# javahedi/SpinDynamics.jl

Hardware: AMD Instinct MI355X
Metric: H|psi> matvecs/s, XXZ L=32 Sz=0 (higher is better)
Workload: dtype c128

## Files before the change

### spindynamics.jl_amd/csrc/kernels_apply.hip

```cpp
#include <hip/hip_runtime.h>

#include <algorithm>
#include <type_traits>

#include "device_common.hpp"


using namespace sd_dev;

namespace {

#ifndef SD_PACK_RING
#define SD_PACK_RING 2
#endif
#ifndef SD_PACK_WGS_PER_CU
#define SD_PACK_WGS_PER_CU 4
#endif
static_assert(SD_PACK_RING >= 2 && SD_PACK_RING <= 4, "ring depth of the packed launch: 2..4 register sets");
static_assert(SD_PACK_WGS_PER_CU >= 2 && SD_PACK_WGS_PER_CU <= 5, "workgroups per CU of the packed launch: 2..5 (95 registers at D = 2)");
template <int NC, int R, int BLOCK, bool FMA, bool PK, bool GEN = false, bool PACK = false>
__global__ __launch_bounds__(BLOCK, (GEN ? 5 : PACK ? SD_PACK_WGS_PER_CU : NC == 2 ? 4 : 5)) void k_apply_tiled(sd_dev_model dm, double *__restrict__ out_,
                                                       const double *__restrict__ psi_, int epi, sd_epi_args ea,
                                                       double *__restrict__ partials, int max_len) {
  using V = typename VT<NC>::type;
  constexpr uint32_t ES = sizeof(V);
  constexpr int WR = R * 64;
  extern __shared__ __attribute__((aligned(16))) unsigned char smem[];
  static_assert(!PACK || (PK && !GEN && R == 4 && BLOCK == 256), "packed launch: four slots of 256 rows, packed tables, chain bonds");
#if SD_PACK_TRACE
  uint64_t trace_t0 = 0;
  if constexpr (PACK) trace_t0 = wall_clock64();
#endif
  constexpr int SLOT_ROWS = WR + 1;
  V *tile = reinterpret_cast<V *>(smem);
  int *lbin = reinterpret_cast<int *>(smem + (size_t)(max_len + 1) * sizeof(V));
  double *red = PACK ? reinterpret_cast<double *>(smem + (size_t)(4 * SLOT_ROWS) * sizeof(V)) : reinterpret_cast<double *>(lbin + 16 * SD_BIN_STRIDE);
  V *tile2 = reinterpret_cast<V *>(red + 32);

  if (ea.batch > 1) {
    const int64_t boff = (int64_t)blockIdx.y * ea.bstride * NC;
    psi_ += boff; out_ += boff;
    if (ea.prev) ea.prev = (const double *)ea.prev + boff;
    if (ea.phi) ea.phi = (const double *)ea.phi + boff;
    if (ea.accv) ea.accv = (double *)ea.accv + boff;
    partials += 2 * (size_t)blockIdx.y * (size_t)dm.n_singles;
    ea.negate = (ea.negate >> blockIdx.y) & 1;
  }
  const V *__restrict__ psi = reinterpret_cast<const V *>(psi_);
  const V *__restrict__ halo = reinterpret_cast<const V *>(ea.halo);
  const int tid = threadIdx.x;
  const int lane = tid & 63;
  int slot_tile = 0, team_wave = 0, team_n = 1, wv = 0;
  bool idle = false;
  if constexpr (PACK) {
    wv = __builtin_amdgcn_readfirstlane(tid >> 6);
    typedef int i4 __attribute__((ext_vector_type(4)));
    const i4 bt = *reinterpret_cast<const i4 *>(dm.blk_tiles + 4 * (size_t)blockIdx.x);
    const int st[4] = {bt.x, bt.y, bt.z, bt.w};
    slot_tile = __builtin_amdgcn_readfirstlane(wv == 0 ? st[0] : wv == 1 ? st[1] : wv == 2 ? st[2] : st[3]);
    team_n = 0;
#pragma unroll
    for (int k = 0; k < 4; ++k) {
      if (st[k] == slot_tile) ++team_n;
      if (st[k] == slot_tile && k < wv) ++team_wave;
    }
    team_wave = __builtin_amdgcn_readfirstlane(team_wave);
    team_n = __builtin_amdgcn_readfirstlane(team_n);
    idle = slot_tile < 0;
    tile += (wv - team_wave) * SLOT_ROWS;
  }
  const int i0 = (PACK ? team_wave : (tid >> 6)) * WR + lane;
  const int tix = PACK ? (idle ? 0 : slot_tile) : blockIdx.x + dm.tile_off;
  const sd_tile_rec rec = dm.single_rec[tix];
  const uint32_t P = rec.prefix;
  const int64_t base = rec.base;
  const int p = dm.p, LS = dm.LS;
  const int len = (PACK && idle) ? 0 : rec.len;
  const int nU = rec.nU;
  const int nn = dm.nn_hops;
  static_assert(!GEN || PK, "general-bond plan: packed tables only");
  const bool need_sig = GEN ? (dm.need_sig_gen != 0) : (!PK || dm.need_sig);

  V own[R];
  uint32_t sig[R];
  typedef unsigned int u4 __attribute__((ext_vector_type(4)));
  u4 pt[PK ? R : 1];
  uint32_t dg[R];
  const uint32_t off0 = (uint32_t)i0 * ES;
  {
    const __amdgpu_buffer_rsrc_t rs = make_rsrc(psi + base, (uint32_t)len * ES);
#pragma unroll
    for (int r = 0; r < R; ++r) buf_load(own[r], rs, off0 + (uint32_t)(r * 64) * ES);
    if (PK && !need_sig && !dm.diag_cache) {
      const __amdgpu_buffer_rsrc_t rg = make_rsrc(dm.suf_dg + rec.suf_off, (uint32_t)len);
#pragma unroll
      for (int r = 0; r < R; ++r) dg[r] = (uint32_t)(unsigned char)__builtin_amdgcn_raw_buffer_load_b8(rg, (uint32_t)i0 + (uint32_t)(r * 64), 0, 0);
    }
    if (need_sig) {
      const __amdgpu_buffer_rsrc_t rsig = make_rsrc(dm.suf_states + rec.suf_off, (uint32_t)len * 2u);
#pragma unroll
      for (int r = 0; r < R; ++r) sig[r] = buf_load_u16(rsig, (uint32_t)i0 * 2u + (uint32_t)(r * 64) * 2u);
    } else {
#pragma unroll
      for (int r = 0; r < R; ++r) sig[r] = 0;
    }
  }

  uint64_t fmask = 0;
  int64_t my_base = -1;
  const uint32_t bitp = p >= 1 ? ((P >> (p - 1)) & 1u) : 0u;
  if (nn > 0 && p >= 1 && !(PACK && idle)) {
    const int b = lane + 1;
    if (b <= p) my_base = dm.far_base[(size_t)tix * (size_t)p + (size_t)lane];
    fmask = __ballot(my_base >= 0);
  }
  const int st_lo = bitp ? nU : 0, st_n = bitp ? len - nU : nU;
  auto get_bond = [&](int ln) {
    FarBond fb;
    fb.base = rl64(my_base, ln); fb.J = dm.hop_J[ln];
    const bool st = ln == p - 1;
    fb.lo = st ? st_lo : 0; fb.n = st ? st_n : len;
    return fb;
  };
  constexpr bool SKIP_DEAD = NC == 1 || BLOCK == 64;
  uint32_t live = 0;
  if (SKIP_DEAD) {
#pragma unroll
    for (int r = 0; r < R; ++r)
      if ((tid & ~63) / 64 * WR + r * 64 < len) live |= 1u << r;
    live = (uint32_t)__builtin_amdgcn_readfirstlane((int)live);
  }
  auto issue = [&](const FarBond &fb, V(&v)[R]) {
    const V *__restrict__ pb = (halo && fb.base >= dm.n_local) ? halo + (fb.base - dm.n_local) : psi + fb.base;
    const __amdgpu_buffer_rsrc_t rs = make_rsrc(pb, (uint32_t)fb.n * ES);
    const uint32_t rel = off0 - (uint32_t)fb.lo * ES;
#pragma unroll
    for (int r = 0; r < R; ++r)
      if (!SKIP_DEAD || ((live >> r) & 1u)) buf_load(v[r], rs, rel + (uint32_t)(r * 64) * ES);
  };

  V va[R], vb[R];
  if (SKIP_DEAD) {
#pragma unroll
    for (int r = 0; r < R; ++r) { va[r] = V{}; vb[r] = V{}; }
  }
  FarBond fa{}, fbb{};
  uint64_t mk = fmask;
  bool have_a = false;
  auto next_lane = [&](uint64_t &m_) { const int ln = __builtin_ctzll(m_); m_ &= m_ - 1; return ln; };
  constexpr int D = PACK ? SD_PACK_RING : 2;
  u4 rq[D][R];
  FarBond fr[D];
  int ring_full = 0, ring_rem = 0;
  auto ring_next = [&]() {
    FarBond fb;
    const bool e = mk == 0;
    const int ln = e ? 0 : __builtin_ctzll(mk);
    mk &= mk - 1;
    fb.base = e ? 0 : rl64(my_base, ln);
    fb.J = 0.0;
    if (!e) fb.J = dm.hop_J[ln];
    const bool st = ln == p - 1;
    fb.lo = st ? st_lo : 0; fb.n = e ? 0 : st ? st_n : len;
    return fb;
  };
  auto ring_issue = [&](const FarBond &fb, u4(&v)[R]) {
    const __amdgpu_buffer_rsrc_t rs = make_rsrc(psi + fb.base, (uint32_t)fb.n * ES);
    const uint32_t rel = off0 - (uint32_t)fb.lo * ES;
#pragma unroll
    for (int r = 0; r < R; ++r) v[r] = __builtin_amdgcn_raw_buffer_load_b128(rs, rel + (uint32_t)(r * 64) * ES, 0, 0);
  };
  auto request_table = [&]() {
    if (PK && (PACK || nn > 0)) {
      const __amdgpu_buffer_rsrc_t rp = make_rsrc(dm.suf_part + 4 * (size_t)rec.suf_off, nn > 0 ? (uint32_t)len * 16u : 0u);
#pragma unroll
      for (int r = 0; r < R; ++r) pt[PK ? r : 0] = __builtin_amdgcn_raw_buffer_load_b128(rp, (uint32_t)i0 * 16u + (uint32_t)(r * 64) * 16u, 0, 0);
    }
  };
  double dd[R];
  auto load_dd = [&]() {
    const __amdgpu_buffer_rsrc_t rd = make_rsrc(dm.diag_cache + base, (uint32_t)len * (uint32_t)sizeof(double));
#pragma unroll
    for (int r = 0; r < R; ++r) buf_load(dd[r], rd, (uint32_t)i0 * (uint32_t)sizeof(double) + (uint32_t)(r * 64) * (uint32_t)sizeof(double));
  };
  if constexpr (PACK) {
    if (dm.diag_cache) load_dd();
    request_table();
    const int nf = __popcll(fmask);
    const int ring_more = nf > D ? nf - D : 0;
    ring_full = ring_more / D;
    ring_rem = ring_more - ring_full * D;
    FarBond fe[D];
#pragma unroll
    for (int j = 0; j < D; ++j) fe[j] = ring_next();
#pragma unroll
    for (int k = 0; k < D; ++k) {
      fr[k] = fe[k];
#pragma unroll
      for (int t = 1; t < D; ++t)
        if (ring_rem == t) fr[k] = fe[(k + t) % D];
      ring_issue(fr[k], rq[k]);
    }
  } else {
    if (mk) { fa = get_bond(next_lane(mk)); issue(fa, va); have_a = true; }
  }

  V acc[R];
  if (dm.diag_cache) {
    if constexpr (!PACK) load_dd();
#pragma unroll
    for (int r = 0; r < R; ++r) acc[r] = vscale(dd[r], own[r]);
  } else if (!need_sig) {
    const int antiP = p >= 2 ? __popc((P ^ (P >> 1)) & ((1u << (p - 1)) - 1u)) : 0;
#pragma unroll
    for (int r = 0; r < R; ++r) {
      int anti = antiP + (int)(dg[r] & 15u) + (p >= 1 ? (int)(bitp ^ (dg[r] >> 4)) : 0);
      if (dm.n_zz_nn == 0) anti = 0;
      acc[r] = vscale(dm.diag_q * (double)(dm.n_zz - 2 * anti), own[r]);
    }
  } else if (dm.diag_mode == 0) {
    const DiagHead dh = diag_head(dm, P, p);
#pragma unroll
    for (int r = 0; r < R; ++r) {
      const uint64_t s = (uint64_t)P | ((uint64_t)sig[r] << p);
      acc[r] = vscale(diag_tail(dm, dh, s, p), own[r]);
    }
  } else {
#pragma unroll
    for (int r = 0; r < R; ++r) {
      const uint64_t s = (uint64_t)P | ((uint64_t)sig[r] << p);
      acc[r] = vscale(diag_of(dm, s), own[r]);
    }
  }
#pragma unroll
  for (int r = 0; r < R; ++r)
    if (i0 + r * 64 < len) tile[1 + i0 + r * 64] = own[r];
  if (PACK ? (lane == 0 && team_wave == 0) : (tid == 0)) tile[0] = V{};
  if (!PK)
    for (int k = tid; k < 16 * SD_BIN_STRIDE; k += BLOCK) {
      int n = k / SD_BIN_STRIDE, kk = k - n * SD_BIN_STRIDE;
      lbin[k] = (int)binom_g(dm, n, kk);
    }

  __syncthreads();
  if constexpr (PACK) {
    auto ring_acc = [&](int k) {
#pragma unroll
      for (int r = 0; r < R; ++r) {
        const u4 q = rq[k][r];
        V v;
        if constexpr (NC == 2) { v.x = __hiloint2double((int)q.y, (int)q.x); v.y = __hiloint2double((int)q.w, (int)q.z); }
        acc[r] = accum<FMA>(acc[r], fr[k].J, v);
      }
    };
    auto ring_step = [&](int k) {
      const FarBond nb = get_bond(next_lane(mk));
      ring_acc(k);
      __builtin_amdgcn_sched_barrier(0);
      fr[k] = nb;
      ring_issue(fr[k], rq[k]);
      __builtin_amdgcn_sched_barrier(0);
    };
#pragma unroll
    for (int k = 1; k < D; ++k)
      if (ring_rem >= D - k) ring_step(k);
#pragma nounroll
    for (int it = 0; it < ring_full; ++it) {
#pragma unroll
      for (int k = 0; k < D; ++k) ring_step(k);
    }
#pragma unroll
    for (int k = 0; k < D; ++k) ring_acc(k);
  } else {
    while (have_a) {
      bool have_b = false;
      if (mk) { fbb = get_bond(next_lane(mk)); issue(fbb, vb); have_b = true; }
#pragma unroll
      for (int r = 0; r < R; ++r) acc[r] = accum<FMA>(acc[r], fa.J, va[r]);
      have_a = false;
      if (!have_b) break;
      if (mk) { fa = get_bond(next_lane(mk)); issue(fa, va); have_a = true; }
#pragma unroll
      for (int r = 0; r < R; ++r) acc[r] = accum<FMA>(acc[r], fbb.J, vb[r]);
    }
  }
  if constexpr (!PACK) request_table();
  const bool wrap = !GEN && !PACK && PK && !(NC == 1 && R == 8) && nn > 0 && dm.wrap_hop == nn;
  bool wrap_on = false;
  if (wrap) {
    const uint32_t Q = P ^ (1u << dm.wrap_pb);
    const int t2q = dm.nup - __popc(Q);
    if (t2q >= 0 && t2q <= LS) {
      wrap_on = true;
      const int64_t qb = dm.addr[Q];
      const int lenq = (int)dm.binom[LS * (SD_MAX_L + 1) + t2q];
      const V *__restrict__ pbq = (halo && qb >= dm.n_local) ? halo + (qb - dm.n_local) : psi + qb;
      const __amdgpu_buffer_rsrc_t rq = make_rsrc(pbq, (uint32_t)lenq * ES);
      for (int c0 = 0; c0 < lenq; c0 += BLOCK * R) {
#pragma unroll
        for (int r = 0; r < R; ++r) buf_load(va[r], rq, off0 + (uint32_t)(c0 + r * 64) * ES);
#pragma unroll
        for (int r = 0; r < R; ++r)
          if (c0 + i0 + r * 64 < lenq) tile2[1 + c0 + i0 + r * 64] = va[r];
      }
      if (tid == 0) tile2[0] = V{};
    }
  }

  struct GBond { int64_t base; uint32_t smask; int pb; int kind; };
  auto gbond = [&](int h) {
    GBond g{0, 0u, 0, -1};
    const int bi = dm.hop_i[h] - 1, bj = dm.hop_j[h] - 1;
    const bool ip = bi < p, jp = bj < p;
    if (ip && jp) {
      if (((P >> bi) ^ (P >> bj)) & 1u) { g.kind = 0; g.base = dm.addr[P ^ (1u << bi) ^ (1u << bj)]; }
    } else if (!ip && !jp) {
      g.kind = 1; g.smask = (1u << (bi - p)) | (1u << (bj - p));
    } else {
      g.pb = ip ? bi : bj;
      g.smask = 1u << ((ip ? bj : bi) - p);
      const uint32_t Q = P ^ (1u << g.pb);
      const int t2q = dm.nup - __popc(Q);
      if (t2q >= 0 && t2q <= LS) { g.kind = 2; g.base = dm.addr[Q]; }
    }
    return g;
  };
  auto gflip = [&](const GBond &g, int r) -> bool {
    if (g.kind == 0) return true;
    if (g.kind == 1) return __popc(sig[r] & g.smask) == 1;
    if (g.kind == 2) return ((P >> g.pb) & 1u) != ((sig[r] & g.smask) ? 1u : 0u);
    return false;
  };
  auto gvalue = [&](const GBond &g, int r) -> V {
    if (g.kind == 1) return tile[1 + dm.suf_rank[sig[r] ^ g.smask]];
    const int64_t idx = g.base + (g.kind == 0 ? (int64_t)(i0 + r * 64) : (int64_t)dm.suf_rank[sig[r] ^ g.smask]);
    return (halo && idx >= dm.n_local) ? halo[idx - dm.n_local] : psi[idx];
  };
  const bool have_g = !GEN && nn < dm.n_hop;
  double gJ = 0.0;
  GBond g0{0, 0u, 0, -1};
  auto request_g0 = [&]() {
    g0 = gbond(nn);
    gJ = dm.hop_J[nn];
#pragma unroll
    for (int r = 0; r < R; ++r) va[r] = (i0 + r * 64 < len && gflip(g0, r)) ? gvalue(g0, r) : V{};
  };
  if (have_g && !PK) request_g0();
  if (nn > 0) {
    if constexpr (PK) {
      const unsigned char *tb = reinterpret_cast<const unsigned char *>(tile);
      constexpr uint32_t SH = NC == 2 ? 4 : 3;
#pragma unroll
      for (int a = 1; a <= 11; ++a) if (a <= LS - 1) {
        const double J = dm.hop_J[p + a - 1];
        const int w = (a - 1) / 3, sh = 10 * ((a - 1) % 3);
        V v[R];
#pragma unroll
        for (int r = 0; r < R; ++r) {
          const u4 q = pt[PK ? r : 0];
          const uint32_t word = w == 0 ? q.x : w == 1 ? q.y : w == 2 ? q.z : q.w;
          const uint32_t ad = ((word >> sh) & 0x3FFu) << SH;
          v[r] = *reinterpret_cast<const V *>(tb + ad);
        }
#pragma unroll
        for (int r = 0; r < R; ++r) acc[r] = accum<FMA>(acc[r], J, v[r]);
      }
    } else {
      uint32_t dw[R];
#pragma unroll
      for (int r = 0; r < R; ++r) dw[r] = sig[r] ^ (sig[r] >> 1);
      for (int a = 1; a <= LS - 1; ++a) {
        const double J = dm.hop_J[p + a - 1];
        const int *brow = lbin + (LS - a - 1) * SD_BIN_STRIDE;
        int d[R];
#pragma unroll
        for (int r = 0; r < R; ++r) d[r] = brow[__popc(sig[r] >> (a + 1))];
        V v[R];
#pragma unroll
        for (int r = 0; r < R; ++r) {
          const bool up = (sig[r] >> (a - 1)) & 1u;
          const bool fl = (dw[r] >> (a - 1)) & 1u;
          const int ip = (i0 + r * 64) + (up ? d[r] : -d[r]);
          v[r] = tile[fl ? ip + 1 : 0];
        }
#pragma unroll
        for (int r = 0; r < R; ++r) acc[r] = accum<FMA>(acc[r], J, v[r]);
      }
    }
  }
  if constexpr (GEN) {
    constexpr uint32_t SH = NC == 2 ? 4 : 3;
    const unsigned char *tb = reinterpret_cast<const unsigned char *>(tile);
    const unsigned char *tb2 = reinterpret_cast<const unsigned char *>(tile2);
    uint32_t ptw[R];
    int cur_word = -1;
    auto gissue = [&](int64_t gbase, V(&v)[R]) {
      const V *__restrict__ pbp = (halo && gbase >= dm.n_local) ? halo + (gbase - dm.n_local) : psi + gbase;
      const __amdgpu_buffer_rsrc_t rs = make_rsrc(pbp, (uint32_t)len * ES);
#pragma unroll
      for (int r = 0; r < R; ++r) buf_load(v[r], rs, off0 + (uint32_t)(r * 64) * ES);
    };
    for (int hb = 0; hb < dm.n_gen; hb += 64) {
      const int nb = dm.n_gen - hb < 64 ? dm.n_gen - hb : 64;
      int64_t base_k = -1;
      sd_gbond gl{-1, 0u, 0, 0, 0.0};
      if (lane < nb) {
        gl = dm.gen[hb + lane];
        if (gl.kind == 0 && __popc(P & gl.pmask) == 1) base_k = dm.addr[P ^ gl.pmask];
      }
      uint64_t todo = __ballot(base_k >= 0);
      int in_a = -1;
      if (todo) { in_a = next_lane(todo); gissue(rl64(base_k, in_a), va); }
#pragma nounroll
      for (int k = 0; k < nb; ++k) {
        sd_gbond gb;
        gb.kind = rl(gl.kind, k); gb.pmask = (uint32_t)rl((int)gl.pmask, k); gb.slot = rl(gl.slot, k); gb.pb = rl(gl.pb, k);
        gb.J = rld(gl.J, k);
        if (gb.kind == 0) {
          if (k == in_a) {
#pragma unroll
            for (int r = 0; r < R; ++r) acc[r] = accum<false>(acc[r], gb.J, va[r]);
            in_a = -1;
            if (todo) { in_a = next_lane(todo); gissue(rl64(base_k, in_a), va); }
          }
        } else if (gb.kind == 1) {
          const int wi = gb.slot / 3, sh = 10 * (gb.slot - 3 * wi);
          if (wi != cur_word) {
            cur_word = wi;
            const int chunk = wi >> 2;
            const __amdgpu_buffer_rsrc_t rp2 = make_rsrc(dm.gen_ss_part + 4 * ((size_t)chunk * (size_t)dm.n_suf_rows + (size_t)rec.suf_off), (uint32_t)len * 16u);
            const uint32_t wo = (uint32_t)(wi & 3) * 4u;
#pragma unroll
            for (int r = 0; r < R; ++r) ptw[r] = (uint32_t)__builtin_amdgcn_raw_buffer_load_b32(rp2, (uint32_t)i0 * 16u + (uint32_t)(r * 64) * 16u + wo, 0, 0);
          }
          V v[R];
#pragma unroll
          for (int r = 0; r < R; ++r) v[r] = *reinterpret_cast<const V *>(tb + ((((ptw[r] >> sh) & 0x3FFu)) << SH));
#pragma unroll
          for (int r = 0; r < R; ++r) acc[r] = accum<false>(acc[r], gb.J, v[r]);
        } else if (gb.kind == 2) {
          const uint32_t Q = P ^ gb.pmask;
          const int t2q = dm.nup - __popc(Q);
          const bool ok = t2q >= 0 && t2q <= LS;
          __syncthreads();
          if (ok) {
            const int64_t qb = dm.addr[Q];
            const int lenq = (int)dm.binom[LS * (SD_MAX_L + 1) + t2q];
            const V *__restrict__ pbq = (halo && qb >= dm.n_local) ? halo + (qb - dm.n_local) : psi + qb;
            const __amdgpu_buffer_rsrc_t rq = make_rsrc(pbq, (uint32_t)lenq * ES);
            for (int c0 = 0; c0 < lenq; c0 += BLOCK * R) {
              V tmp[R];
#pragma unroll
              for (int r = 0; r < R; ++r) buf_load(tmp[r], rq, off0 + (uint32_t)(c0 + r * 64) * ES);
#pragma unroll
              for (int r = 0; r < R; ++r)
                if (c0 + i0 + r * 64 < lenq) tile2[1 + c0 + i0 + r * 64] = tmp[r];
            }
            if (tid == 0) tile2[0] = V{};
          }
          __syncthreads();
          if (ok) {
            const __amdgpu_buffer_rsrc_t rm = make_rsrc(dm.mix_part + ((size_t)gb.slot * (size_t)dm.n_suf_rows + (size_t)rec.suf_off), (uint32_t)len * 2u);
            const uint32_t bpb = (P >> gb.pb) & 1u;
            uint32_t w16[R];
#pragma unroll
            for (int r = 0; r < R; ++r) w16[r] = buf_load_u16(rm, (uint32_t)i0 * 2u + (uint32_t)(r * 64) * 2u);
#pragma unroll
            for (int r = 0; r < R; ++r) {
              const bool has = (w16[r] >> 15) != bpb;
              const uint32_t ad = has ? ((w16[r] & 0x3FFu) << SH) : 0u;
              acc[r] = accum<false>(acc[r], gb.J, *reinterpret_cast<const V *>(tb2 + ad));
            }
          }
        }
      }
    }
  }
  if (wrap) {
    __syncthreads();
    if (wrap_on) {
      const double Jw = dm.hop_J[nn];
      const uint32_t bpb = (P >> dm.wrap_pb) & 1u;
      const unsigned char *tb2 = reinterpret_cast<const unsigned char *>(tile2);
      constexpr uint32_t SH = NC == 2 ? 4 : 3;
#pragma unroll
      for (int r = 0; r < R; ++r) {
        const uint32_t w3 = pt[PK ? r : 0].w;
        const bool has = ((w3 >> 30) & 1u) != bpb;
        const uint32_t ad = has ? (((w3 >> 20) & 0x3FFu) << SH) : 0u;
        acc[r] = accum<false>(acc[r], Jw, *reinterpret_cast<const V *>(tb2 + ad));
      }
    }
  }
  if (have_g) {
    if (!wrap) {
      if (PK) request_g0();
#pragma unroll
      for (int r = 0; r < R; ++r)
        if (gflip(g0, r)) acc[r] = accum<false>(acc[r], gJ, va[r]);
    }
    for (int h = nn + 1; h < dm.n_hop; ++h) {
      const GBond g = gbond(h);
      if (g.kind < 0) continue;
      const double J = dm.hop_J[h];
#pragma unroll
      for (int r = 0; r < R; ++r)
        if (i0 + r * 64 < len && gflip(g, r)) acc[r] = accum<false>(acc[r], J, gvalue(g, r));
    }
  }

  EpiSums sums{0.0, 0.0};
#pragma unroll
  for (int r = 0; r < R; ++r) {
    const int i = i0 + r * 64;
    if (i < len) epilogue<NC>(epi, ea, base + i, acc[r], tile[1 + i], out_, sums);
  }
  if (epi_has_sums(epi)) {
    double a = sums.s0, b = sums.s1;
    if constexpr (PACK) {
      for (int off = 32; off > 0; off >>= 1) {
        a += __shfl_down(a, off, 64);
        b += __shfl_down(b, off, 64);
      }
      if (lane == 0) { red[2 * wv] = a; red[2 * wv + 1] = b; }
      __syncthreads();
      if (lane == 0 && team_wave == 0 && !idle) {
        double x = 0.0, y = 0.0;
        for (int w = 0; w < team_n; ++w) { x += red[2 * (wv + w)]; y += red[2 * (wv + w) + 1]; }
        partials[2 * (size_t)tix] = x; partials[2 * (size_t)tix + 1] = y;
      }
    } else {
      block_reduce2(a, b, red);
      if (tid == 0) { partials[2 * (size_t)tix] = a; partials[2 * (size_t)tix + 1] = b; }
    }
  }
#if SD_PACK_TRACE
  if constexpr (PACK) {
    if (dm.pack_trace && tid == 0 && blockIdx.y == 0) {
      __builtin_amdgcn_s_waitcnt(0);
      uint64_t *rec_t = dm.pack_trace + 3 * (size_t)blockIdx.x;
      rec_t[0] = trace_t0;
      rec_t[1] = wall_clock64();
      rec_t[2] = (uint64_t)(__builtin_amdgcn_s_getreg((3 << 11) | 20) & 15u);
    }
  }
#endif
}

template <int NC, bool FMA>
__global__ __launch_bounds__(256, 4) void k_apply_fulltile(sd_dev_model dm, double *__restrict__ out_,
                                                        const double *__restrict__ psi_, int epi, sd_epi_args ea,
                                                        double *__restrict__ partials) {
  using V = typename VT<NC>::type;
  constexpr uint32_t ES = sizeof(V);
  constexpr int R = 4, BLOCK = 256;
  extern __shared__ __attribute__((aligned(16))) unsigned char smem[];
  const int LF = dm.full_ls, TL = 1 << LF;
  V *tile = reinterpret_cast<V *>(smem);
  double *red = reinterpret_cast<double *>(smem + (size_t)(TL + 1) * sizeof(V));
  const V *__restrict__ psi = reinterpret_cast<const V *>(psi_);
  const V *__restrict__ halo = reinterpret_cast<const V *>(ea.halo);
  const int tid = threadIdx.x, lane = tid & 63;
  uint32_t T = blockIdx.x;
  if (gridDim.x >= 512 && (gridDim.x & 255u) == 0) {
    const uint32_t x = T & 7u, j = T >> 3, g = j >> 5, i = j & 31u;
    T = (g << 8) + (x << 5) + i;
  }
  const int64_t base = (int64_t)T << LF;
  const uint32_t Tg = T + (uint32_t)(dm.row_lo >> LF);
  const int64_t gbase = (int64_t)Tg << LF;
  const int nn = dm.nn_hops;

  V own[R];
  uint32_t ioff[R];
  {
    const __amdgpu_buffer_rsrc_t rs = make_rsrc(psi + base, (uint32_t)TL * ES);
#pragma unroll
    for (int r = 0; r < R; ++r) { ioff[r] = (uint32_t)(tid + r * BLOCK) * ES; buf_load(own[r], rs, ioff[r]); }
  }
  uint64_t fmask = 0;
  int64_t my_base = 0;
  double my_J = 0.0;
  int my_lo = 0, my_n = TL;
  if (nn > 0) {
    const int a = LF + lane;
    bool fl = false;
    if (a <= dm.L - 1) {
      if (lane == 0) {
        const int t = (int)(T & 1u);
        my_lo = (1 - t) * (TL / 2); my_n = TL / 2;
        my_base = ((int64_t)(T ^ 1u) << LF) + (TL / 2 - my_lo);
        fl = true;
      } else {
        const int b = a - LF - 1;
        fl = ((Tg >> b) ^ (Tg >> (b + 1))) & 1u;
        const uint32_t Tp = Tg ^ (3u << b);
        const int tb = dm.L - LF - dm.fs_dbits;
        const uint32_t q = Tp >> tb;
        const int64_t at_peer = (int64_t)(Tp & ((1u << tb) - 1u)) << LF;
        my_base = at_peer;
        if (q != (Tg >> tb)) {
          int64_t ho = 0, plo = 0;
#pragma unroll
          for (int q2 = 0; q2 < SD_FS_MAX_RANKS; ++q2)
            if ((uint32_t)q2 == q) { ho = dm.fs_halo_off[q2]; plo = dm.fs_peer_lo[q2]; }
          my_base = dm.n_local + ho + at_peer - plo;
        }
      }
      my_J = dm.hop_J[a - 1];
    }
    fmask = __ballot(fl);
  }
  auto get_bond = [&](int ln) {
    FarBond fb;
    fb.base = rl64(my_base, ln); fb.J = rld(my_J, ln);
    fb.lo = rl(my_lo, ln); fb.n = rl(my_n, ln);
    return fb;
  };
  auto issue = [&](const FarBond &fb, V(&v)[R]) {
    const V *__restrict__ pb = (halo && fb.base >= dm.n_local) ? halo + (fb.base - dm.n_local) : psi + fb.base;
    const __amdgpu_buffer_rsrc_t rs = make_rsrc(pb, (uint32_t)fb.n * ES);
    const uint32_t lo_b = (uint32_t)fb.lo * ES;
#pragma unroll
    for (int r = 0; r < R; ++r) buf_load(v[r], rs, ioff[r] - lo_b);
  };
  V va[R], vb[R];
  FarBond fa{}, fbb{};
  uint64_t mk = fmask;
  bool have_a = false;
  auto next_lane = [&](uint64_t &m_) { const int ln = __builtin_ctzll(m_); m_ &= m_ - 1; return ln; };
  if (mk) { fa = get_bond(next_lane(mk)); issue(fa, va); have_a = true; }

  V acc[R];
#pragma unroll
  for (int r = 0; r < R; ++r) {
    acc[r] = vscale(diag_of(dm, (uint64_t)gbase + (uint64_t)(tid + r * BLOCK)), own[r]);
    tile[tid + r * BLOCK] = own[r];
  }
  if (tid == 0) tile[TL] = V{};
  __syncthreads();

  const int n_in = nn > 0 ? LF - 1 : 0;
  for (int a = 1; a <= n_in; ++a) {
    const double J = dm.hop_J[a - 1];
    V v[R];
#pragma unroll
    for (int r = 0; r < R; ++r) {
      const int i = tid + r * BLOCK;
      const bool fl = ((i >> (a - 1)) ^ (i >> a)) & 1;
      v[r] = tile[fl ? (i ^ (3 << (a - 1))) : TL];
    }
#pragma unroll
    for (int r = 0; r < R; ++r) acc[r] = accum<FMA>(acc[r], J, v[r]);
  }
  while (have_a) {
    bool have_b = false;
    if (mk) { fbb = get_bond(next_lane(mk)); issue(fbb, vb); have_b = true; }
#pragma unroll
    for (int r = 0; r < R; ++r) acc[r] = accum<FMA>(acc[r], fa.J, va[r]);
    have_a = false;
    if (!have_b) break;
    if (mk) { fa = get_bond(next_lane(mk)); issue(fa, va); have_a = true; }
#pragma unroll
    for (int r = 0; r < R; ++r) acc[r] = accum<FMA>(acc[r], fbb.J, vb[r]);
  }
  for (int h = nn; h < dm.n_hop; ++h) {
    const int bi = dm.hop_i[h] - 1, bj = dm.hop_j[h] - 1;
    const double J = dm.hop_J[h];
#pragma unroll
    for (int r = 0; r < R; ++r) {
      const uint64_t s = (uint64_t)gbase + (uint64_t)(tid + r * BLOCK);
      if (((s >> bi) ^ (s >> bj)) & 1) acc[r] = accum<false>(acc[r], J, psi[s ^ ((uint64_t)1 << bi) ^ ((uint64_t)1 << bj)]);
    }
  }
  EpiSums sums{0.0, 0.0};
#pragma unroll
  for (int r = 0; r < R; ++r) {
    const int i = tid + r * BLOCK;
    epilogue<NC>(epi, ea, base + i, acc[r], tile[i], out_, sums);
  }
  if (epi_has_sums(epi)) {
    double a = sums.s0, b = sums.s1;
    block_reduce2(a, b, red);
    if (tid == 0) { partials[2 * (size_t)blockIdx.x] = a; partials[2 * (size_t)blockIdx.x + 1] = b; }
  }
}

template <int NC>
__global__ __launch_bounds__(256) void k_apply_generic(sd_dev_model dm, double *__restrict__ out_,
                                                       const double *__restrict__ psi_, int epi, sd_epi_args ea,
                                                       double *__restrict__ partials) {
  using V = typename VT<NC>::type;
  __shared__ double red[32];
  __shared__ int64_t lb[64 * 64];
  const V *__restrict__ psi = reinterpret_cast<const V *>(psi_);
  const bool full = dm.nup < 0;
  const int L = dm.L;
  if (!full) {
    for (int i = threadIdx.x; i < 64 * 64; i += blockDim.x) {
      const int n = i >> 6, k = i & 63;
      lb[i] = (n <= L && k <= n) ? dm.binom[n * (SD_MAX_L + 1) + k] : 0;
    }
    __syncthreads();
  }
  auto bl = [&](int n, int k) -> int64_t { return (k < 0 || k > n) ? 0 : lb[(n << 6) + k]; };
  auto unrank_l = [&](int64_t idx) {
    uint64_t s = 0;
    int r = dm.nup;
    for (int k = 1; k <= L && r > 0; ++k) {
      const int64_t c = bl(L - k, r - 1);
      if (idx < c) { s |= (uint64_t)1 << (k - 1); --r; }
      else idx -= c;
    }
    return s;
  };
  auto rank_l = [&](uint64_t s) {
    int64_t idx = 0;
    int r = dm.nup;
    for (int k = 1; k <= L && r > 0; ++k) {
      if ((s >> (k - 1)) & 1) --r;
      else idx += bl(L - k, r - 1);
    }
    return idx;
  };
  const int nn = full ? 0 : dm.nn_hops;
  EpiSums sums{0.0, 0.0};
  const int64_t stride = (int64_t)gridDim.x * blockDim.x;
  for (int64_t idx = (int64_t)blockIdx.x * blockDim.x + threadIdx.x; idx < dm.N; idx += stride) {
    const uint64_t s = full ? (uint64_t)idx : unrank_l(idx);
    const V own = psi[idx];
    V acc = vscale(diag_of(dm, s), own);
    for (int b = 1; b <= nn; ++b)
      if (((s >> (b - 1)) ^ (s >> b)) & 1) {
        const int64_t d = lb[((L - b - 1) << 6) + __popcll(s >> (b + 1))];
        const int64_t nidx = ((s >> (b - 1)) & 1) ? idx + d : idx - d;
        acc = vadd_mul(acc, dm.hop_J[b - 1], psi[nidx]);
      }
    for (int h = nn; h < dm.n_hop; ++h) {
      const int bi = dm.hop_i[h] - 1, bj = dm.hop_j[h] - 1;
      if (((s >> bi) ^ (s >> bj)) & 1) {
        const uint64_t s2 = s ^ ((uint64_t)1 << bi) ^ ((uint64_t)1 << bj);
        const int64_t nidx = full ? (int64_t)s2 : rank_l(s2);
        acc = vadd_mul(acc, dm.hop_J[h], psi[nidx]);
      }
    }
    epilogue<NC>(epi, ea, idx, acc, own, out_, sums);
  }
  if (epi_has_sums(epi)) {
    double a = sums.s0, b = sums.s1;
    block_reduce2(a, b, red);
    if (threadIdx.x == 0) { partials[2 * (size_t)blockIdx.x] = a; partials[2 * (size_t)blockIdx.x + 1] = b; }
  }
}

template <int NC, int LPT>
__global__ __launch_bounds__(256) void k_apply_short(sd_dev_model dm, double *__restrict__ out_, const double *__restrict__ psi_, int epi,
                                                     sd_epi_args ea, double *__restrict__ partials, int first, int count) {
  using V = typename VT<NC>::type;
  __shared__ int64_t lb[64 * 64];
  if (ea.batch > 1) {
    const int64_t boff = (int64_t)blockIdx.y * ea.bstride * NC;
    psi_ += boff; out_ += boff;
    if (ea.prev) ea.prev = (const double *)ea.prev + boff;
    if (ea.phi) ea.phi = (const double *)ea.phi + boff;
    if (ea.accv) ea.accv = (double *)ea.accv + boff;
    partials += 2 * (size_t)blockIdx.y * (size_t)dm.n_singles;
    ea.negate = (ea.negate >> blockIdx.y) & 1;
  }
  const V *__restrict__ psi = reinterpret_cast<const V *>(psi_);
  const int L = dm.L, p = dm.p;
  for (int i = threadIdx.x; i < 64 * 64; i += blockDim.x) {
    const int n = i >> 6, k = i & 63;
    lb[i] = (n <= L && k <= n) ? dm.binom[n * (SD_MAX_L + 1) + k] : 0;
  }
  __syncthreads();
  auto bl = [&](int n, int k) -> int64_t { return (k < 0 || k > n) ? 0 : lb[(n << 6) + k]; };
  auto rank_l = [&](uint64_t s) {
    int64_t idx = 0;
    int r = dm.nup;
    for (int k = 1; k <= L && r > 0; ++k) {
      if ((s >> (k - 1)) & 1) --r;
      else idx += bl(L - k, r - 1);
    }
    return idx;
  };
  constexpr int TPB = 256 / LPT;
  const int i = threadIdx.x % LPT;
  const int nn = dm.nn_hops;
  const int sweeps = (count + (int)gridDim.x * TPB - 1) / ((int)gridDim.x * TPB);
  for (int sw = 0; sw < sweeps; ++sw) {
    const int g = (sw * (int)gridDim.x + (int)blockIdx.x) * TPB + (int)threadIdx.x / LPT;
    const bool have_tile = g < count;
    const int tix = first + (have_tile ? g : 0);
    const sd_tile_rec rec = dm.single_rec[tix];
    EpiSums sums{0.0, 0.0};
    if (have_tile && i < rec.len) {
      const int64_t idx = rec.base + i;
      const uint64_t s = (uint64_t)rec.prefix | ((uint64_t)dm.suf_states[rec.suf_off + i] << p);
      const V own = psi[idx];
      V acc = vscale(dm.diag_cache ? dm.diag_cache[idx] : diag_of(dm, s), own);
      for (int b = 1; b <= nn; ++b)
        if (((s >> (b - 1)) ^ (s >> b)) & 1) {
          const int64_t d = lb[((L - b - 1) << 6) + __popcll(s >> (b + 1))];
          const int64_t nidx = ((s >> (b - 1)) & 1) ? idx + d : idx - d;
          acc = vadd_mul(acc, dm.hop_J[b - 1], psi[nidx]);
        }
      for (int h = nn; h < dm.n_hop; ++h) {
        const int bi = dm.hop_i[h] - 1, bj = dm.hop_j[h] - 1;
        if (((s >> bi) ^ (s >> bj)) & 1) {
          const uint64_t s2 = s ^ ((uint64_t)1 << bi) ^ ((uint64_t)1 << bj);
          acc = vadd_mul(acc, dm.hop_J[h], psi[rank_l(s2)]);
        }
      }
      epilogue<NC>(epi, ea, idx, acc, own, out_, sums);
    }
    if (epi_has_sums(epi)) {
      double a = sums.s0, b = sums.s1;
      if (LPT > 1)
        for (int off = LPT / 2; off > 0; off >>= 1) {
          a += __shfl_down(a, off, LPT);
          b += __shfl_down(b, off, LPT);
        }
      if (have_tile && i == 0) { partials[2 * (size_t)tix] = a; partials[2 * (size_t)tix + 1] = b; }
    }
  }
}

template <int NC>
__global__ __launch_bounds__(256) void k_epilogue_only(int epi, sd_epi_args ea, int64_t n, double *out_,
                                                       const double *hpsi_, const double *__restrict__ psi_,
                                                       double *__restrict__ partials) {
  using V = typename VT<NC>::type;
  __shared__ double red[32];
  const V *hpsi = reinterpret_cast<const V *>(hpsi_);
  const V *__restrict__ psi = reinterpret_cast<const V *>(psi_);
  EpiSums sums{0.0, 0.0};
  const int64_t stride = (int64_t)gridDim.x * blockDim.x;
  for (int64_t i = (int64_t)blockIdx.x * blockDim.x + threadIdx.x; i < n; i += stride) {
    const V acc = hpsi[i], own = psi[i];
    epilogue<NC>(epi, ea, i, acc, own, out_, sums);
  }
  if (epi_has_sums(epi)) {
    double a = sums.s0, b = sums.s1;
    block_reduce2(a, b, red);
    if (threadIdx.x == 0) { partials[2 * (size_t)blockIdx.x] = a; partials[2 * (size_t)blockIdx.x + 1] = b; }
  }
}

__global__ __launch_bounds__(1024) void k_reduce_pairs(const double *__restrict__ partials, int64_t n,
                                                       double *__restrict__ scalars, int64_t dstride) {
  __shared__ double red[32];
  partials += 2 * (size_t)blockIdx.x * (size_t)n;
  scalars += (size_t)blockIdx.x * (size_t)dstride;
  double a = 0.0, b = 0.0;
  for (int64_t i = threadIdx.x; i < n; i += blockDim.x) { a += partials[2 * i]; b += partials[2 * i + 1]; }
  block_reduce2(a, b, red);
  if (threadIdx.x == 0) { scalars[0] = a; scalars[1] = b; }
}

__global__ __launch_bounds__(256) void k_reduce_pairs_stage(const double *__restrict__ partials, int64_t n, int64_t chunk,
                                                            double *__restrict__ stage) {
  __shared__ double red[32];
  const int64_t lo = (int64_t)blockIdx.x * chunk, hi = lo + chunk < n ? lo + chunk : n;
  const double2 *__restrict__ p2 = reinterpret_cast<const double2 *>(partials);
  double a = 0.0, b = 0.0;
  for (int64_t i = lo + threadIdx.x; i < hi; i += blockDim.x) { const double2 v = p2[i]; a += v.x; b += v.y; }
  block_reduce2(a, b, red);
  if (threadIdx.x == 0) { stage[2 * blockIdx.x] = a; stage[2 * blockIdx.x + 1] = b; }
}

}
int sd_reduce_pairs(sd_ctx *ctx, int64_t n, double *dst) {
  if (!dst) dst = ctx->d_scalars;
  const double *src = ctx->d_partials;
  if (n > 16384) {
    double *stage = ctx->d_partials + 2 * n;
    const int64_t chunk = (n + SD_RED_STAGE_BLOCKS - 1) / SD_RED_STAGE_BLOCKS;
    hipLaunchKernelGGL(k_reduce_pairs_stage, dim3(SD_RED_STAGE_BLOCKS), dim3(256), 0, ctx->stream, src, n, chunk, stage);
    SD_HIP(ctx, hipGetLastError());
    src = stage; n = SD_RED_STAGE_BLOCKS;
  }
  hipLaunchKernelGGL(k_reduce_pairs, dim3(1), dim3(1024), 0, ctx->stream, src, n, dst, (int64_t)0);
  SD_HIP(ctx, hipGetLastError());
  return SD_OK;
}
int sd_reduce_pairs_batched(sd_ctx *ctx, int64_t n, int batch, double *dst, int64_t dstride) {
  if (!dst || n > 16384 || batch < 1) return sd_set_err(ctx, SD_EINTERNAL, "bad batched reduction");
  hipLaunchKernelGGL(k_reduce_pairs, dim3((unsigned)batch), dim3(1024), 0, ctx->stream, ctx->d_partials, n, dst, dstride);
  SD_HIP(ctx, hipGetLastError());
  return SD_OK;
}
int sd_launch_epilogue_only(sd_ctx *ctx, int dtype, int64_t n, void *out, const void *hpsi, const void *psi, int epi,
                            const sd_epi_args &ea_in) {
  const bool sums = (epi == SD_EPI_DOT || epi == SD_EPI_KPM || epi == SD_EPI_RESCALE_DOT);
  sd_epi_args ea = ea_in;
  ea.stream_hint = 0;
  if (n <= 0) {
    if (sums) SD_HIP(ctx, hipMemsetAsync(ea.sums_dst ? ea.sums_dst : ctx->d_scalars, 0, 2 * sizeof(double), ctx->stream));
    return SD_OK;
  }
  const int64_t nb = std::min<int64_t>((n + 255) / 256, 4096);
  if (sums) { int rc = sd_ensure_partials(ctx, 2 * (size_t)nb + 2 * SD_RED_STAGE_BLOCKS); if (rc) return rc; }
  if (dtype == SD_C128)
    hipLaunchKernelGGL(k_epilogue_only<2>, dim3((unsigned)nb), dim3(256), 0, ctx->stream, epi, ea, n, (double *)out,
                       (const double *)hpsi, (const double *)psi, ctx->d_partials);
  else
    hipLaunchKernelGGL(k_epilogue_only<1>, dim3((unsigned)nb), dim3(256), 0, ctx->stream, epi, ea, n, (double *)out,
                       (const double *)hpsi, (const double *)psi, ctx->d_partials);
  SD_HIP(ctx, hipGetLastError());
  if (sums) return sd_reduce_pairs(ctx, nb, ea.sums_dst);
  return SD_OK;
}
namespace {

template <int NC, int R, int BLOCK, bool FMA, bool PK, bool GEN = false, bool PACK = false>
int launch_tiled_cfg(sd_ctx *ctx, const sd_dev_model &dm, int nt, size_t shmem, double *out, const double *psi, int epi,
                     const sd_epi_args &ea, int max_len) {
  void (*kern)(sd_dev_model, double *, const double *, int, sd_epi_args, double *, int) = k_apply_tiled<NC, R, BLOCK, FMA, PK, GEN, PACK>;
  if (shmem > 48 * 1024)
    SD_HIP(ctx, hipFuncSetAttribute((const void *)kern, hipFuncAttributeMaxDynamicSharedMemorySize, (int)shmem));
  hipLaunchKernelGGL(kern, dim3(nt, ea.batch > 1 ? ea.batch : 1), dim3(BLOCK), shmem, ctx->stream, dm, out, psi, epi, ea, ctx->d_partials, max_len);
  SD_HIP(ctx, hipGetLastError());
  return SD_OK;
}

template <int NC, bool FMA>
int launch_tiled(sd_ctx *ctx, const sd_dev_model &dm, int nt, int cls, size_t shmem, double *out, const double *psi, int epi,
                 const sd_epi_args &ea, int max_len) {
  constexpr int R = 4;
  if ((64 << cls) * R < max_len) return sd_set_err(ctx, SD_EINTERNAL, "tile longer than its workgroup can hold");
  if (!dm.suf_part) {
    switch (cls) {
      case 3: return launch_tiled_cfg<NC, R, 512, FMA, false>(ctx, dm, nt, shmem, out, psi, epi, ea, max_len);
      case 4: return launch_tiled_cfg<NC, R, 1024, FMA, false>(ctx, dm, nt, shmem, out, psi, epi, ea, max_len);
    }
    return sd_set_err(ctx, SD_EINTERNAL, "bad tile length class for a plan without the packed partner table");
  }
  if (dm.n_gen > 0)
    switch (cls) {
      case 0: return launch_tiled_cfg<NC, R, 64, FMA, true, true>(ctx, dm, nt, shmem, out, psi, epi, ea, max_len);
      case 1: return launch_tiled_cfg<NC, R, 128, FMA, true, true>(ctx, dm, nt, shmem, out, psi, epi, ea, max_len);
      case 2: return launch_tiled_cfg<NC, R, 256, FMA, true, true>(ctx, dm, nt, shmem, out, psi, epi, ea, max_len);
      default: return sd_set_err(ctx, SD_EINTERNAL, "bad tile length class");
    }
  constexpr bool F8 = NC == 1;
  switch (cls) {
    case 0: return launch_tiled_cfg<NC, R, 64, FMA, true>(ctx, dm, nt, shmem, out, psi, epi, ea, max_len);
    case 1: return launch_tiled_cfg<NC, F8 ? 8 : R, F8 ? 64 : 128, FMA, true>(ctx, dm, nt, shmem, out, psi, epi, ea, max_len);
    case 2: return launch_tiled_cfg<NC, F8 ? 8 : R, F8 ? 128 : 256, FMA, true>(ctx, dm, nt, shmem, out, psi, epi, ea, max_len);
  }
  return sd_set_err(ctx, SD_EINTERNAL, "bad tile length class");
}

}

int sd_launch_apply(sd_ctx *ctx, const sd_model *m, int dtype, void *out, const void *psi, int epi,
                    const sd_epi_args &ea_in, int part) {
  if (!m->dev_ready) return sd_set_err(ctx, SD_EARG, "model has no device tables (created without a context)");
  if (dtype != SD_F64 && dtype != SD_C128) return sd_set_err(ctx, SD_EARG, "dtype must be SD_F64 or SD_C128");
  const bool sums = (epi == SD_EPI_DOT || epi == SD_EPI_KPM || epi == SD_EPI_RESCALE_DOT);
  sd_dev_model dm = m->dm;
  sd_epi_args ea = ea_in;
  ea.stream_hint = 3;
  if (dm.n_local == 0) {
    if (sums) SD_HIP(ctx, hipMemsetAsync(ea.sums_dst ? ea.sums_dst : ctx->d_scalars, 0, 2 * sizeof(double), ctx->stream));
    return SD_OK;
  }
  if (ea.no_reduce && (m->p < 0 || part != 0)) return sd_set_err(ctx, SD_EINTERNAL, "unreduced sums: whole tiled plans only");
  if (ea.batch > 1 && (m->p < 0 || m->nranks != 1 || part != 0 || dm.n_singles > 16384 || (sums && !ea.sums_dst && !ea.no_reduce)))
    return sd_set_err(ctx, SD_EINTERNAL, "batched apply: unsharded tiled plans with at most 16384 tiles only");
  if (m->p >= 0) {
    int nt = dm.n_singles;
    if (part == 1) nt = dm.n_interior;
    else if (part == 2) nt = dm.n_singles - dm.n_interior;
    if (sums) { int rc = sd_ensure_partials(ctx, 2 * (size_t)dm.n_singles * (size_t)std::max(ea.batch, 1) + 2 * SD_RED_STAGE_BLOCKS); if (rc) return rc; }
    const int max_len = m->max_tile_len;
    const size_t esz = dtype == SD_C128 ? 16 : 8;
    int rc = SD_OK;
    if (nt > 0) {
      const bool packed = part == 0 && dtype == SD_C128 && dm.n_blk > 0;
      if (packed) {
        constexpr size_t LDS_CU = 160 * 1024, WGS = SD_PACK_WGS_PER_CU;
        const size_t need = (size_t)4 * 257 * esz + 32 * sizeof(double) + 16;
        const size_t shmem = WGS >= 6 ? need : std::max(need, ((LDS_CU / WGS + LDS_CU / (WGS + 1)) / 2) & ~(size_t)255);
        rc = m->hop_pow2 ? launch_tiled_cfg<2, 4, 256, true, true, false, true>(ctx, dm, dm.n_blk, shmem, (double *)out, (const double *)psi, epi, ea, 1024)
                         : launch_tiled_cfg<2, 4, 256, false, true, false, true>(ctx, dm, dm.n_blk, shmem, (double *)out, (const double *)psi, epi, ea, 1024);
      }
      const int s0 = part == 2 ? SD_N_LEN_CLASS : 0, s1 = packed ? s0 : part == 1 ? SD_N_LEN_CLASS : 2 * SD_N_LEN_CLASS;
      for (int sg = s0; sg < s1 && rc == SD_OK; ++sg) {
        const int cnt = m->seg_off[sg + 1] - m->seg_off[sg];
        if (cnt <= 0) continue;
        const int cls = m->seg_cls[sg];
        const int seg_max = std::min(max_len, (64 << cls) * 4);
        size_t shmem = (size_t)(seg_max + 1) * esz + 16 * SD_BIN_STRIDE * sizeof(int) + 32 * sizeof(double) + 16;
        if ((dm.wrap_hop >= 0 && dm.wrap_hop == dm.nn_hops) || dm.n_gen_mixed > 0) shmem += (size_t)(m->max_tile_len_all + 1) * esz;
        dm.tile_off = m->seg_off[sg];
        if (dtype == SD_C128)
          rc = m->hop_pow2 ? launch_tiled<2, true>(ctx, dm, cnt, cls, shmem, (double *)out, (const double *)psi, epi, ea, seg_max)
                           : launch_tiled<2, false>(ctx, dm, cnt, cls, shmem, (double *)out, (const double *)psi, epi, ea, seg_max);
        else
          rc = m->hop_pow2 ? launch_tiled<1, true>(ctx, dm, cnt, cls, shmem, (double *)out, (const double *)psi, epi, ea, seg_max)
                           : launch_tiled<1, false>(ctx, dm, cnt, cls, shmem, (double *)out, (const double *)psi, epi, ea, seg_max);
      }
      if (rc) return rc;
      if (dm.n_short > 0 && part == 0) {
        const unsigned by = ea.batch > 1 ? (unsigned)ea.batch : 1u;
        auto blocks = [](int tiles, int per_block) { return (unsigned)std::min(4096, std::max(1, (tiles + per_block - 1) / per_block)); };
        const int n16 = dm.n_short_multi, n1 = dm.n_short - dm.n_short_multi;
        if (n16 > 0) {
          if (dtype == SD_C128) hipLaunchKernelGGL((k_apply_short<2, 16>), dim3(blocks(n16, 16), by), dim3(256), 0, ctx->stream, dm, (double *)out, (const double *)psi, epi, ea, ctx->d_partials, dm.short_off, n16);
          else hipLaunchKernelGGL((k_apply_short<1, 16>), dim3(blocks(n16, 16), by), dim3(256), 0, ctx->stream, dm, (double *)out, (const double *)psi, epi, ea, ctx->d_partials, dm.short_off, n16);
        }
        if (n1 > 0) {
          if (dtype == SD_C128) hipLaunchKernelGGL((k_apply_short<2, 1>), dim3(blocks(n1, 256), by), dim3(256), 0, ctx->stream, dm, (double *)out, (const double *)psi, epi, ea, ctx->d_partials, dm.short_off + n16, n1);
          else hipLaunchKernelGGL((k_apply_short<1, 1>), dim3(blocks(n1, 256), by), dim3(256), 0, ctx->stream, dm, (double *)out, (const double *)psi, epi, ea, ctx->d_partials, dm.short_off + n16, n1);
        }
        SD_HIP(ctx, hipGetLastError());
      }
    }
    if (sums && part != 1 && !ea.no_reduce) {
      int rc2 = ea.batch > 1 ? sd_reduce_pairs_batched(ctx, (int64_t)dm.n_singles, ea.batch, ea.sums_dst, ea.sums_bstride)
                             : sd_reduce_pairs(ctx, (int64_t)dm.n_singles, ea.sums_dst);
      if (rc2) return rc2;
    }
  } else if (m->full_ls > 0) {
    if (part == 1) return SD_OK;
    const int64_t nb = dm.n_local >> m->full_ls;
    if (sums) { int rc = sd_ensure_partials(ctx, 2 * (size_t)nb + 2 * SD_RED_STAGE_BLOCKS); if (rc) return rc; }
    const size_t esz = dtype == SD_C128 ? 16 : 8;
    const size_t shmem = (((size_t)1 << m->full_ls) + 1) * esz + 32 * sizeof(double) + 16;
    void (*kf)(sd_dev_model, double *, const double *, int, sd_epi_args, double *) =
        dtype == SD_C128 ? (m->hop_pow2 ? k_apply_fulltile<2, true> : k_apply_fulltile<2, false>)
                         : (m->hop_pow2 ? k_apply_fulltile<1, true> : k_apply_fulltile<1, false>);
    hipLaunchKernelGGL(kf, dim3((unsigned)nb), dim3(256), shmem, ctx->stream, dm, (double *)out, (const double *)psi, epi, ea,
                       ctx->d_partials);
    SD_HIP(ctx, hipGetLastError());
    if (sums) {
      int rc2 = sd_reduce_pairs(ctx, (int64_t)nb, ea.sums_dst);
      if (rc2) return rc2;
    }
  } else {
    int64_t nb = (dm.N + 255) / 256;
    if (nb > 8192) nb = 8192;
    if (sums) { int rc = sd_ensure_partials(ctx, 2 * (size_t)nb + 2 * SD_RED_STAGE_BLOCKS); if (rc) return rc; }
    if (dtype == SD_C128)
      hipLaunchKernelGGL(k_apply_generic<2>, dim3((unsigned)nb), dim3(256), 0, ctx->stream, dm, (double *)out,
                         (const double *)psi, epi, ea, ctx->d_partials);
    else
      hipLaunchKernelGGL(k_apply_generic<1>, dim3((unsigned)nb), dim3(256), 0, ctx->stream, dm, (double *)out,
                         (const double *)psi, epi, ea, ctx->d_partials);
    SD_HIP(ctx, hipGetLastError());
    if (sums) {
      int rc2 = sd_reduce_pairs(ctx, (int64_t)nb, ea.sums_dst);
      if (rc2) return rc2;
    }
  }
  return SD_OK;
}
```

Before: 105.6.

## Specialize packed tiled kernel body by live row-group count per wave

The tiled kernel body now lives in a self-included section, so it can be instantiated several times with a compile-time row count R. In the packed launch, each wave computes how many 64-row groups of its slot are live and dispatches to a body with R=4 or R=2 (or R=3, depending on SD_PACK_BODIES). This avoids issuing loads and accumulations for dead row groups. Hop amplitudes in the packed path are also read through the constant address space. The cost is larger code and possible divergence in register allocation between bodies, plus some added compile complexity.

```diff
diff --git a/profiles/live_groups.py b/profiles/live_groups.py
--- /dev/null
+++ b/profiles/live_groups.py
@@ -0,0 +1,141 @@
+#!/usr/bin/env python3
+import os
+import sys
+from collections import Counter
+from math import comb
+
+sys.path.insert(0, os.path.dirname(os.path.abspath(__file__)))
+from orbit_key import deal, orbit_key, tile_costs
+
+QUAD_BLOCKS, CAP_TENTHS, DEAL_COST, RUN = 2, 78, "slots", 3
+RING = 2
+SLOT_GROUPS, GROUP_ROWS = 4, 64
+
+
+def tile_len(P, nup, LS):
+    t = nup - bin(P).count("1")
+    return comb(LS, t) if 0 <= t <= LS else 0
+
+
+def tile_base(P, L, p, nup):
+    idx, r = 0, nup
+    for k in range(1, p + 1):
+        if r <= 0:
+            break
+        if (P >> (k - 1)) & 1:
+            r -= 1
+        else:
+            idx += comb(L - k, r - 1)
+    return idx
+
+
+def list_length(P, p, nup, LS):
+    n = bin((P ^ (P >> 1)) & ((1 << (p - 1)) - 1)).count("1") if p >= 2 else 0
+    t = nup - bin(P).count("1")
+    bitp = (P >> (p - 1)) & 1
+    tq = t + 1 if bitp else t - 1
+    nU = comb(LS - 1, t - 1) if t >= 1 else 0
+    mine = comb(LS, t) - nU if bitp else nU
+    return n + (1 if 0 <= tq <= LS and mine > 0 else 0)
+
+
+def queues(L, nup, LS=12):
+    p = L - LS
+    tiles = sorted((P for P in range(1 << p) if tile_len(P, nup, LS) > 0), key=lambda P: tile_base(P, L, p, nup))
+    first, keys = {}, []
+    for P in tiles:
+        rep, mem, _ = orbit_key(P, p, QUAD_BLOCKS, CAP_TENTHS)
+        keys.append((first.setdefault(rep, len(first)), mem))
+    idx = sorted(range(len(tiles)), key=lambda k: keys[k])
+    orbits, members = [], []
+    for k in idx:
+        if not members or keys[k][0] != keys[members[-1][0]][0]:
+            members.append([])
+            orbits.append([0, 0, 0, 0, 0])
+        members[-1].append(k)
+        orbits[-1][0] += 1
+        for n, c in enumerate(tile_costs(tiles[k], p, LS, nup, QUAD_BLOCKS, CAP_TENTHS)):
+            orbits[-1][1 + n] += c
+    q = [[] for _ in range(8)]
+    for mem, x in zip(members, deal([tuple(o) for o in orbits], DEAL_COST, RUN)):
+        q[x].extend(tiles[k] for k in mem)
+    return q
+
+
+def blocks(L, nup, LS=12):
+    out = []
+    for queue in queues(L, nup, LS):
+        cur = []
+        for P in queue:
+            s = (tile_len(P, nup, LS) + 255) // 256
+            if len(cur) + s > 4:
+                out.append(tuple(cur + [-1] * (4 - len(cur))))
+                cur = []
+            cur += [P] * s
+        if cur:
+            out.append(tuple(cur + [-1] * (4 - len(cur))))
+    return out
+
+
+def waves(L, nup, LS=12):
+    p = L - LS
+    out = []
+    for blk in blocks(L, nup, LS):
+        for w, P in enumerate(blk):
+            if P < 0:
+                out.append((0, 0, 0))
+                continue
+            team_wave = w - blk.index(P)
+            ln = tile_len(P, nup, LS)
+            live = min(SLOT_GROUPS, max(0, -(-(ln - team_wave * SLOT_GROUPS * GROUP_ROWS) // GROUP_ROWS)))
+            out.append((ln, live, list_length(P, p, nup, LS)))
+    return out
+
+
+def groups_run(live, bodies):
+    live = max(live, 1)
+    return SLOT_GROUPS if bodies == 1 else live if bodies == 4 else (2 if live <= 2 else 4)
+
+
+def vmem_reads(ln, live, nf, bodies):
+    g = groups_run(live, bodies)
+    return (3 + max(nf, RING)) * g + (1 if ln > 0 else 0)
+
+
+def count(L, nup, LS=12):
+    ws = waves(L, nup, LS)
+    by_len = {}
+    for ln, live, _ in ws:
+        if ln == 0:
+            continue
+        t = by_len.setdefault(ln, [0, 0, 0])
+        t[1] += SLOT_GROUPS
+        t[2] += live
+    for ln, t in by_len.items():
+        t[0] = t[1] // (SLOT_GROUPS * ((ln + 255) // 256))
+    return {"by_len": {ln: tuple(t) for ln, t in by_len.items()},
+            "idle": sum(1 for w in ws if w[0] == 0),
+            "body": Counter(max(w[1], 1) for w in ws),
+            "groups": {b: sum(groups_run(w[1], b) for w in ws) for b in (1, 2, 4)},
+            "vmem": {b: sum(vmem_reads(*w, b) for w in ws) for b in (1, 2, 4)}}
+
+
+if __name__ == "__main__":
+    L = int(sys.argv[1]) if len(sys.argv) > 1 else 32
+    nup = int(sys.argv[2]) if len(sys.argv) > 2 else L // 2
+    LS = int(sys.argv[3]) if len(sys.argv) > 3 else 12
+    c = count(L, nup, LS)
+    print(f"L={L} nup={nup} LS={LS}: packed launch, {sum(c['body'].values())} wave slots, {c['idle']} idle")
+    print("| tile rows | slots | groups issued / live per tile | tiles | dead groups |")
+    print("|---:|---:|---:|---:|---:|")
+    for ln in sorted(c["by_len"], reverse=True):
+        tiles, issued, live = c["by_len"][ln]
+        print(f"| {ln} | {(ln + 255) // 256} | {issued // tiles} / {live // tiles} | {tiles} | {issued - live} |")
+    issued = sum(t[1] for t in c["by_len"].values())
+    live = sum(t[2] for t in c["by_len"].values())
+    print(f"row groups of tiles: {issued} issued, {live} live, {issued - live} dead ({100.0 * (issued - live) / issued:.2f} %);"
+          f" idle slots add {SLOT_GROUPS * c['idle']} issued groups before, {c['idle']} now")
+    print("waves by live groups (idle slots under 1):", dict(sorted(c["body"].items())))
+    for b, name in ((1, "before (every wave four groups)"), (4, "four bodies"), (2, "two bodies (<= 2, 4)")):
+        print(f"{name:34s}: {c['groups'][b]:>10d} groups run, {c['vmem'][b]:>11d} vector-memory read wave-instructions"
+              f" ({100.0 * (c['vmem'][b] - c['vmem'][1]) / c['vmem'][1]:+.2f} %)")
diff --git a/spindynamics.jl_amd/csrc/kernels_apply.hip b/spindynamics.jl_amd/csrc/kernels_apply.hip
--- a/spindynamics.jl_amd/csrc/kernels_apply.hip
+++ b/spindynamics.jl_amd/csrc/kernels_apply.hip
@@ -1,3 +1,4 @@
+#ifndef SD_TILED_BODY_PASS
 #include <hip/hip_runtime.h>
 
 #include <algorithm>
@@ -16,17 +17,26 @@
 #ifndef SD_PACK_WGS_PER_CU
 #define SD_PACK_WGS_PER_CU 4
 #endif
+template <bool CONST_AS>
+__device__ __forceinline__ double hop_amp(const double *__restrict__ J, int h) {
+  if constexpr (CONST_AS) return ((const __attribute__((address_space(4))) double *)J)[h];
+  else return J[h];
+}
+#ifndef SD_PACK_BODIES
+#define SD_PACK_BODIES 2
+#endif
+static_assert(SD_PACK_BODIES == 1 || SD_PACK_BODIES == 2 || SD_PACK_BODIES == 4, "bodies of the packed launch: 1, 2 or 4");
 static_assert(SD_PACK_RING >= 2 && SD_PACK_RING <= 4, "ring depth of the packed launch: 2..4 register sets");
 static_assert(SD_PACK_WGS_PER_CU >= 2 && SD_PACK_WGS_PER_CU <= 5, "workgroups per CU of the packed launch: 2..5 (95 registers at D = 2)");
-template <int NC, int R, int BLOCK, bool FMA, bool PK, bool GEN = false, bool PACK = false>
+template <int NC, int RW, int BLOCK, bool FMA, bool PK, bool GEN = false, bool PACK = false>
 __global__ __launch_bounds__(BLOCK, (GEN ? 5 : PACK ? SD_PACK_WGS_PER_CU : NC == 2 ? 4 : 5)) void k_apply_tiled(sd_dev_model dm, double *__restrict__ out_,
                                                        const double *__restrict__ psi_, int epi, sd_epi_args ea,
                                                        double *__restrict__ partials, int max_len) {
   using V = typename VT<NC>::type;
   constexpr uint32_t ES = sizeof(V);
-  constexpr int WR = R * 64;
+  constexpr int WR = RW * 64;
   extern __shared__ __attribute__((aligned(16))) unsigned char smem[];
-  static_assert(!PACK || (PK && !GEN && R == 4 && BLOCK == 256), "packed launch: four slots of 256 rows, packed tables, chain bonds");
+  static_assert(!PACK || (PK && !GEN && RW == 4 && BLOCK == 256), "packed launch: four slots of 256 rows, packed tables, chain bonds");
 #if SD_PACK_TRACE
   uint64_t trace_t0 = 0;
   if constexpr (PACK) trace_t0 = wall_clock64();
@@ -81,459 +91,28 @@
   static_assert(!GEN || PK, "general-bond plan: packed tables only");
   const bool need_sig = GEN ? (dm.need_sig_gen != 0) : (!PK || dm.need_sig);
 
-  V own[R];
-  uint32_t sig[R];
-  typedef unsigned int u4 __attribute__((ext_vector_type(4)));
-  u4 pt[PK ? R : 1];
-  uint32_t dg[R];
-  const uint32_t off0 = (uint32_t)i0 * ES;
-  {
-    const __amdgpu_buffer_rsrc_t rs = make_rsrc(psi + base, (uint32_t)len * ES);
-#pragma unroll
-    for (int r = 0; r < R; ++r) buf_load(own[r], rs, off0 + (uint32_t)(r * 64) * ES);
-    if (PK && !need_sig && !dm.diag_cache) {
-      const __amdgpu_buffer_rsrc_t rg = make_rsrc(dm.suf_dg + rec.suf_off, (uint32_t)len);
-#pragma unroll
-      for (int r = 0; r < R; ++r) dg[r] = (uint32_t)(unsigned char)__builtin_amdgcn_raw_buffer_load_b8(rg, (uint32_t)i0 + (uint32_t)(r * 64), 0, 0);
-    }
-    if (need_sig) {
-      const __amdgpu_buffer_rsrc_t rsig = make_rsrc(dm.suf_states + rec.suf_off, (uint32_t)len * 2u);
-#pragma unroll
-      for (int r = 0; r < R; ++r) sig[r] = buf_load_u16(rsig, (uint32_t)i0 * 2u + (uint32_t)(r * 64) * 2u);
+#define SD_TILED_BODY_PASS 1
+  if constexpr (!PACK) {
+    constexpr int R = RW;
+#include "kernels_apply.hip"
+  } else {
+    int n_live = (len - team_wave * WR + 63) >> 6;
+    n_live = __builtin_amdgcn_readfirstlane(n_live < 1 ? 1 : n_live > RW ? RW : n_live);
+    if (SD_PACK_BODIES == 1 || n_live == 4 || (SD_PACK_BODIES == 2 && n_live == 3)) {
+      constexpr int R = 4;
+#include "kernels_apply.hip"
+    } else if (SD_PACK_BODIES == 4 && n_live == 3) {
+      constexpr int R = 3;
+#include "kernels_apply.hip"
+    } else if (SD_PACK_BODIES == 2 || n_live == 2) {
+      constexpr int R = 2;
+#include "kernels_apply.hip"
     } else {
-#pragma unroll
-      for (int r = 0; r < R; ++r) sig[r] = 0;
-    }
-  }
-
-  uint64_t fmask = 0;
-  int64_t my_base = -1;
-  const uint32_t bitp = p >= 1 ? ((P >> (p - 1)) & 1u) : 0u;
-  if (nn > 0 && p >= 1 && !(PACK && idle)) {
-    const int b = lane + 1;
-    if (b <= p) my_base = dm.far_base[(size_t)tix * (size_t)p + (size_t)lane];
-    fmask = __ballot(my_base >= 0);
-  }
-  const int st_lo = bitp ? nU : 0, st_n = bitp ? len - nU : nU;
-  auto get_bond = [&](int ln) {
-    FarBond fb;
-    fb.base = rl64(my_base, ln); fb.J = dm.hop_J[ln];
-    const bool st = ln == p - 1;
-    fb.lo = st ? st_lo : 0; fb.n = st ? st_n : len;
-    return fb;
-  };
-  constexpr bool SKIP_DEAD = NC == 1 || BLOCK == 64;
-  uint32_t live = 0;
-  if (SKIP_DEAD) {
-#pragma unroll
-    for (int r = 0; r < R; ++r)
-      if ((tid & ~63) / 64 * WR + r * 64 < len) live |= 1u << r;
-    live = (uint32_t)__builtin_amdgcn_readfirstlane((int)live);
-  }
-  auto issue = [&](const FarBond &fb, V(&v)[R]) {
-    const V *__restrict__ pb = (halo && fb.base >= dm.n_local) ? halo + (fb.base - dm.n_local) : psi + fb.base;
-    const __amdgpu_buffer_rsrc_t rs = make_rsrc(pb, (uint32_t)fb.n * ES);
-    const uint32_t rel = off0 - (uint32_t)fb.lo * ES;
-#pragma unroll
-    for (int r = 0; r < R; ++r)
-      if (!SKIP_DEAD || ((live >> r) & 1u)) buf_load(v[r], rs, rel + (uint32_t)(r * 64) * ES);
-  };
-
-  V va[R], vb[R];
-  if (SKIP_DEAD) {
-#pragma unroll
-    for (int r = 0; r < R; ++r) { va[r] = V{}; vb[r] = V{}; }
-  }
-  FarBond fa{}, fbb{};
-  uint64_t mk = fmask;
-  bool have_a = false;
-  auto next_lane = [&](uint64_t &m_) { const int ln = __builtin_ctzll(m_); m_ &= m_ - 1; return ln; };
-  constexpr int D = PACK ? SD_PACK_RING : 2;
-  u4 rq[D][R];
-  FarBond fr[D];
-  int ring_full = 0, ring_rem = 0;
-  auto ring_next = [&]() {
-    FarBond fb;
-    const bool e = mk == 0;
-    const int ln = e ? 0 : __builtin_ctzll(mk);
-    mk &= mk - 1;
-    fb.base = e ? 0 : rl64(my_base, ln);
-    fb.J = 0.0;
-    if (!e) fb.J = dm.hop_J[ln];
-    const bool st = ln == p - 1;
-    fb.lo = st ? st_lo : 0; fb.n = e ? 0 : st ? st_n : len;
-    return fb;
-  };
-  auto ring_issue = [&](const FarBond &fb, u4(&v)[R]) {
-    const __amdgpu_buffer_rsrc_t rs = make_rsrc(psi + fb.base, (uint32_t)fb.n * ES);
-    const uint32_t rel = off0 - (uint32_t)fb.lo * ES;
-#pragma unroll
-    for (int r = 0; r < R; ++r) v[r] = __builtin_amdgcn_raw_buffer_load_b128(rs, rel + (uint32_t)(r * 64) * ES, 0, 0);
-  };
-  auto request_table = [&]() {
-    if (PK && (PACK || nn > 0)) {
-      const __amdgpu_buffer_rsrc_t rp = make_rsrc(dm.suf_part + 4 * (size_t)rec.suf_off, nn > 0 ? (uint32_t)len * 16u : 0u);
-#pragma unroll
-      for (int r = 0; r < R; ++r) pt[PK ? r : 0] = __builtin_amdgcn_raw_buffer_load_b128(rp, (uint32_t)i0 * 16u + (uint32_t)(r * 64) * 16u, 0, 0);
-    }
-  };
-  double dd[R];
-  auto load_dd = [&]() {
-    const __amdgpu_buffer_rsrc_t rd = make_rsrc(dm.diag_cache + base, (uint32_t)len * (uint32_t)sizeof(double));
-#pragma unroll
-    for (int r = 0; r < R; ++r) buf_load(dd[r], rd, (uint32_t)i0 * (uint32_t)sizeof(double) + (uint32_t)(r * 64) * (uint32_t)sizeof(double));
-  };
-  if constexpr (PACK) {
-    if (dm.diag_cache) load_dd();
-    request_table();
-    const int nf = __popcll(fmask);
-    const int ring_more = nf > D ? nf - D : 0;
-    ring_full = ring_more / D;
-    ring_rem = ring_more - ring_full * D;
-    FarBond fe[D];
-#pragma unroll
-    for (int j = 0; j < D; ++j) fe[j] = ring_next();
-#pragma unroll
-    for (int k = 0; k < D; ++k) {
-      fr[k] = fe[k];
-#pragma unroll
-      for (int t = 1; t < D; ++t)
-        if (ring_rem == t) fr[k] = fe[(k + t) % D];
-      ring_issue(fr[k], rq[k]);
-    }
-  } else {
-    if (mk) { fa = get_bond(next_lane(mk)); issue(fa, va); have_a = true; }
-  }
-
-  V acc[R];
-  if (dm.diag_cache) {
-    if constexpr (!PACK) load_dd();
-#pragma unroll
-    for (int r = 0; r < R; ++r) acc[r] = vscale(dd[r], own[r]);
-  } else if (!need_sig) {
-    const int antiP = p >= 2 ? __popc((P ^ (P >> 1)) & ((1u << (p - 1)) - 1u)) : 0;
-#pragma unroll
-    for (int r = 0; r < R; ++r) {
-      int anti = antiP + (int)(dg[r] & 15u) + (p >= 1 ? (int)(bitp ^ (dg[r] >> 4)) : 0);
-      if (dm.n_zz_nn == 0) anti = 0;
-      acc[r] = vscale(dm.diag_q * (double)(dm.n_zz - 2 * anti), own[r]);
-    }
-  } else if (dm.diag_mode == 0) {
-    const DiagHead dh = diag_head(dm, P, p);
-#pragma unroll
-    for (int r = 0; r < R; ++r) {
-      const uint64_t s = (uint64_t)P | ((uint64_t)sig[r] << p);
-      acc[r] = vscale(diag_tail(dm, dh, s, p), own[r]);
-    }
-  } else {
-#pragma unroll
-    for (int r = 0; r < R; ++r) {
-      const uint64_t s = (uint64_t)P | ((uint64_t)sig[r] << p);
-      acc[r] = vscale(diag_of(dm, s), own[r]);
-    }
-  }
-#pragma unroll
-  for (int r = 0; r < R; ++r)
-    if (i0 + r * 64 < len) tile[1 + i0 + r * 64] = own[r];
-  if (PACK ? (lane == 0 && team_wave == 0) : (tid == 0)) tile[0] = V{};
-  if (!PK)
-    for (int k = tid; k < 16 * SD_BIN_STRIDE; k += BLOCK) {
-      int n = k / SD_BIN_STRIDE, kk = k - n * SD_BIN_STRIDE;
-      lbin[k] = (int)binom_g(dm, n, kk);
-    }
-
-  __syncthreads();
-  if constexpr (PACK) {
-    auto ring_acc = [&](int k) {
-#pragma unroll
-      for (int r = 0; r < R; ++r) {
-        const u4 q = rq[k][r];
-        V v;
-        if constexpr (NC == 2) { v.x = __hiloint2double((int)q.y, (int)q.x); v.y = __hiloint2double((int)q.w, (int)q.z); }
-        acc[r] = accum<FMA>(acc[r], fr[k].J, v);
-      }
-    };
-    auto ring_step = [&](int k) {
-      const FarBond nb = get_bond(next_lane(mk));
-      ring_acc(k);
-      __builtin_amdgcn_sched_barrier(0);
-      fr[k] = nb;
-      ring_issue(fr[k], rq[k]);
-      __builtin_amdgcn_sched_barrier(0);
-    };
-#pragma unroll
-    for (int k = 1; k < D; ++k)
-      if (ring_rem >= D - k) ring_step(k);
-#pragma nounroll
-    for (int it = 0; it < ring_full; ++it) {
-#pragma unroll
-      for (int k = 0; k < D; ++k) ring_step(k);
-    }
-#pragma unroll
-    for (int k = 0; k < D; ++k) ring_acc(k);
-  } else {
-    while (have_a) {
-      bool have_b = false;
-      if (mk) { fbb = get_bond(next_lane(mk)); issue(fbb, vb); have_b = true; }
-#pragma unroll
-      for (int r = 0; r < R; ++r) acc[r] = accum<FMA>(acc[r], fa.J, va[r]);
-      have_a = false;
-      if (!have_b) break;
-      if (mk) { fa = get_bond(next_lane(mk)); issue(fa, va); have_a = true; }
-#pragma unroll
-      for (int r = 0; r < R; ++r) acc[r] = accum<FMA>(acc[r], fbb.J, vb[r]);
-    }
-  }
-  if constexpr (!PACK) request_table();
-  const bool wrap = !GEN && !PACK && PK && !(NC == 1 && R == 8) && nn > 0 && dm.wrap_hop == nn;
-  bool wrap_on = false;
-  if (wrap) {
-    const uint32_t Q = P ^ (1u << dm.wrap_pb);
-    const int t2q = dm.nup - __popc(Q);
-    if (t2q >= 0 && t2q <= LS) {
-      wrap_on = true;
-      const int64_t qb = dm.addr[Q];
-      const int lenq = (int)dm.binom[LS * (SD_MAX_L + 1) + t2q];
-      const V *__restrict__ pbq = (halo && qb >= dm.n_local) ? halo + (qb - dm.n_local) : psi + qb;
-      const __amdgpu_buffer_rsrc_t rq = make_rsrc(pbq, (uint32_t)lenq * ES);
-      for (int c0 = 0; c0 < lenq; c0 += BLOCK * R) {
-#pragma unroll
-        for (int r = 0; r < R; ++r) buf_load(va[r], rq, off0 + (uint32_t)(c0 + r * 64) * ES);
-#pragma unroll
-        for (int r = 0; r < R; ++r)
-          if (c0 + i0 + r * 64 < lenq) tile2[1 + c0 + i0 + r * 64] = va[r];
-      }
-      if (tid == 0) tile2[0] = V{};
-    }
-  }
-
-  struct GBond { int64_t base; uint32_t smask; int pb; int kind; };
-  auto gbond = [&](int h) {
-    GBond g{0, 0u, 0, -1};
-    const int bi = dm.hop_i[h] - 1, bj = dm.hop_j[h] - 1;
-    const bool ip = bi < p, jp = bj < p;
-    if (ip && jp) {
-      if (((P >> bi) ^ (P >> bj)) & 1u) { g.kind = 0; g.base = dm.addr[P ^ (1u << bi) ^ (1u << bj)]; }
-    } else if (!ip && !jp) {
-      g.kind = 1; g.smask = (1u << (bi - p)) | (1u << (bj - p));
-    } else {
-      g.pb = ip ? bi : bj;
-      g.smask = 1u << ((ip ? bj : bi) - p);
-      const uint32_t Q = P ^ (1u << g.pb);
-      const int t2q = dm.nup - __popc(Q);
-      if (t2q >= 0 && t2q <= LS) { g.kind = 2; g.base = dm.addr[Q]; }
-    }
-    return g;
-  };
-  auto gflip = [&](const GBond &g, int r) -> bool {
-    if (g.kind == 0) return true;
-    if (g.kind == 1) return __popc(sig[r] & g.smask) == 1;
-    if (g.kind == 2) return ((P >> g.pb) & 1u) != ((sig[r] & g.smask) ? 1u : 0u);
-    return false;
-  };
-  auto gvalue = [&](const GBond &g, int r) -> V {
-    if (g.kind == 1) return tile[1 + dm.suf_rank[sig[r] ^ g.smask]];
-    const int64_t idx = g.base + (g.kind == 0 ? (int64_t)(i0 + r * 64) : (int64_t)dm.suf_rank[sig[r] ^ g.smask]);
-    return (halo && idx >= dm.n_local) ? halo[idx - dm.n_local] : psi[idx];
-  };
-  const bool have_g = !GEN && nn < dm.n_hop;
-  double gJ = 0.0;
-  GBond g0{0, 0u, 0, -1};
-  auto request_g0 = [&]() {
-    g0 = gbond(nn);
-    gJ = dm.hop_J[nn];
-#pragma unroll
-    for (int r = 0; r < R; ++r) va[r] = (i0 + r * 64 < len && gflip(g0, r)) ? gvalue(g0, r) : V{};
-  };
-  if (have_g && !PK) request_g0();
-  if (nn > 0) {
-    if constexpr (PK) {
-      const unsigned char *tb = reinterpret_cast<const unsigned char *>(tile);
-      constexpr uint32_t SH = NC == 2 ? 4 : 3;
-#pragma unroll
-      for (int a = 1; a <= 11; ++a) if (a <= LS - 1) {
-        const double J = dm.hop_J[p + a - 1];
-        const int w = (a - 1) / 3, sh = 10 * ((a - 1) % 3);
-        V v[R];
-#pragma unroll
-        for (int r = 0; r < R; ++r) {
-          const u4 q = pt[PK ? r : 0];
-          const uint32_t word = w == 0 ? q.x : w == 1 ? q.y : w == 2 ? q.z : q.w;
-          const uint32_t ad = ((word >> sh) & 0x3FFu) << SH;
-          v[r] = *reinterpret_cast<const V *>(tb + ad);
-        }
-#pragma unroll
-        for (int r = 0; r < R; ++r) acc[r] = accum<FMA>(acc[r], J, v[r]);
-      }
-    } else {
-      uint32_t dw[R];
-#pragma unroll
-      for (int r = 0; r < R; ++r) dw[r] = sig[r] ^ (sig[r] >> 1);
-      for (int a = 1; a <= LS - 1; ++a) {
-        const double J = dm.hop_J[p + a - 1];
-        const int *brow = lbin + (LS - a - 1) * SD_BIN_STRIDE;
-        int d[R];
-#pragma unroll
-        for (int r = 0; r < R; ++r) d[r] = brow[__popc(sig[r] >> (a + 1))];
-        V v[R];
-#pragma unroll
-        for (int r = 0; r < R; ++r) {
-          const bool up = (sig[r] >> (a - 1)) & 1u;
-          const bool fl = (dw[r] >> (a - 1)) & 1u;
-          const int ip = (i0 + r * 64) + (up ? d[r] : -d[r]);
-          v[r] = tile[fl ? ip + 1 : 0];
-        }
-#pragma unroll
-        for (int r = 0; r < R; ++r) acc[r] = accum<FMA>(acc[r], J, v[r]);
-      }
-    }
-  }
-  if constexpr (GEN) {
-    constexpr uint32_t SH = NC == 2 ? 4 : 3;
-    const unsigned char *tb = reinterpret_cast<const unsigned char *>(tile);
-    const unsigned char *tb2 = reinterpret_cast<const unsigned char *>(tile2);
-    uint32_t ptw[R];
-    int cur_word = -1;
-    auto gissue = [&](int64_t gbase, V(&v)[R]) {
-      const V *__restrict__ pbp = (halo && gbase >= dm.n_local) ? halo + (gbase - dm.n_local) : psi + gbase;
-      const __amdgpu_buffer_rsrc_t rs = make_rsrc(pbp, (uint32_t)len * ES);
-#pragma unroll
-      for (int r = 0; r < R; ++r) buf_load(v[r], rs, off0 + (uint32_t)(r * 64) * ES);
-    };
-    for (int hb = 0; hb < dm.n_gen; hb += 64) {
-      const int nb = dm.n_gen - hb < 64 ? dm.n_gen - hb : 64;
-      int64_t base_k = -1;
-      sd_gbond gl{-1, 0u, 0, 0, 0.0};
-      if (lane < nb) {
-        gl = dm.gen[hb + lane];
-        if (gl.kind == 0 && __popc(P & gl.pmask) == 1) base_k = dm.addr[P ^ gl.pmask];
-      }
-      uint64_t todo = __ballot(base_k >= 0);
-      int in_a = -1;
-      if (todo) { in_a = next_lane(todo); gissue(rl64(base_k, in_a), va); }
-#pragma nounroll
-      for (int k = 0; k < nb; ++k) {
-        sd_gbond gb;
-        gb.kind = rl(gl.kind, k); gb.pmask = (uint32_t)rl((int)gl.pmask, k); gb.slot = rl(gl.slot, k); gb.pb = rl(gl.pb, k);
-        gb.J = rld(gl.J, k);
-        if (gb.kind == 0) {
-          if (k == in_a) {
-#pragma unroll
-            for (int r = 0; r < R; ++r) acc[r] = accum<false>(acc[r], gb.J, va[r]);
-            in_a = -1;
-            if (todo) { in_a = next_lane(todo); gissue(rl64(base_k, in_a), va); }
-          }
-        } else if (gb.kind == 1) {
-          const int wi = gb.slot / 3, sh = 10 * (gb.slot - 3 * wi);
-          if (wi != cur_word) {
-            cur_word = wi;
-            const int chunk = wi >> 2;
-            const __amdgpu_buffer_rsrc_t rp2 = make_rsrc(dm.gen_ss_part + 4 * ((size_t)chunk * (size_t)dm.n_suf_rows + (size_t)rec.suf_off), (uint32_t)len * 16u);
-            const uint32_t wo = (uint32_t)(wi & 3) * 4u;
-#pragma unroll
-            for (int r = 0; r < R; ++r) ptw[r] = (uint32_t)__builtin_amdgcn_raw_buffer_load_b32(rp2, (uint32_t)i0 * 16u + (uint32_t)(r * 64) * 16u + wo, 0, 0);
-          }
-          V v[R];
-#pragma unroll
-          for (int r = 0; r < R; ++r) v[r] = *reinterpret_cast<const V *>(tb + ((((ptw[r] >> sh) & 0x3FFu)) << SH));
-#pragma unroll
-          for (int r = 0; r < R; ++r) acc[r] = accum<false>(acc[r], gb.J, v[r]);
-        } else if (gb.kind == 2) {
-          const uint32_t Q = P ^ gb.pmask;
-          const int t2q = dm.nup - __popc(Q);
-          const bool ok = t2q >= 0 && t2q <= LS;
-          __syncthreads();
-          if (ok) {
-            const int64_t qb = dm.addr[Q];
-            const int lenq = (int)dm.binom[LS * (SD_MAX_L + 1) + t2q];
-            const V *__restrict__ pbq = (halo && qb >= dm.n_local) ? halo + (qb - dm.n_local) : psi + qb;
-            const __amdgpu_buffer_rsrc_t rq = make_rsrc(pbq, (uint32_t)lenq * ES);
-            for (int c0 = 0; c0 < lenq; c0 += BLOCK * R) {
-              V tmp[R];
-#pragma unroll
-              for (int r = 0; r < R; ++r) buf_load(tmp[r], rq, off0 + (uint32_t)(c0 + r * 64) * ES);
-#pragma unroll
-              for (int r = 0; r < R; ++r)
-                if (c0 + i0 + r * 64 < lenq) tile2[1 + c0 + i0 + r * 64] = tmp[r];
-            }
-            if (tid == 0) tile2[0] = V{};
-          }
-          __syncthreads();
-          if (ok) {
-            const __amdgpu_buffer_rsrc_t rm = make_rsrc(dm.mix_part + ((size_t)gb.slot * (size_t)dm.n_suf_rows + (size_t)rec.suf_off), (uint32_t)len * 2u);
-            const uint32_t bpb = (P >> gb.pb) & 1u;
-            uint32_t w16[R];
-#pragma unroll
-            for (int r = 0; r < R; ++r) w16[r] = buf_load_u16(rm, (uint32_t)i0 * 2u + (uint32_t)(r * 64) * 2u);
-#pragma unroll
-            for (int r = 0; r < R; ++r) {
-              const bool has = (w16[r] >> 15) != bpb;
-              const uint32_t ad = has ? ((w16[r] & 0x3FFu) << SH) : 0u;
-              acc[r] = accum<false>(acc[r], gb.J, *reinterpret_cast<const V *>(tb2 + ad));
-            }
-          }
-        }
-      }
-    }
-  }
-  if (wrap) {
-    __syncthreads();
-    if (wrap_on) {
-      const double Jw = dm.hop_J[nn];
-      const uint32_t bpb = (P >> dm.wrap_pb) & 1u;
-      const unsigned char *tb2 = reinterpret_cast<const unsigned char *>(tile2);
-      constexpr uint32_t SH = NC == 2 ? 4 : 3;
-#pragma unroll
-      for (int r = 0; r < R; ++r) {
-        const uint32_t w3 = pt[PK ? r : 0].w;
-        const bool has = ((w3 >> 30) & 1u) != bpb;
-        const uint32_t ad = has ? (((w3 >> 20) & 0x3FFu) << SH) : 0u;
-        acc[r] = accum<false>(acc[r], Jw, *reinterpret_cast<const V *>(tb2 + ad));
-      }
-    }
-  }
-  if (have_g) {
-    if (!wrap) {
-      if (PK) request_g0();
-#pragma unroll
-      for (int r = 0; r < R; ++r)
-        if (gflip(g0, r)) acc[r] = accum<false>(acc[r], gJ, va[r]);
-    }
-    for (int h = nn + 1; h < dm.n_hop; ++h) {
-      const GBond g = gbond(h);
-      if (g.kind < 0) continue;
-      const double J = dm.hop_J[h];
-#pragma unroll
-      for (int r = 0; r < R; ++r)
-        if (i0 + r * 64 < len && gflip(g, r)) acc[r] = accum<false>(acc[r], J, gvalue(g, r));
-    }
-  }
-
-  EpiSums sums{0.0, 0.0};
-#pragma unroll
-  for (int r = 0; r < R; ++r) {
-    const int i = i0 + r * 64;
-    if (i < len) epilogue<NC>(epi, ea, base + i, acc[r], tile[1 + i], out_, sums);
-  }
-  if (epi_has_sums(epi)) {
-    double a = sums.s0, b = sums.s1;
-    if constexpr (PACK) {
-      for (int off = 32; off > 0; off >>= 1) {
-        a += __shfl_down(a, off, 64);
-        b += __shfl_down(b, off, 64);
-      }
-      if (lane == 0) { red[2 * wv] = a; red[2 * wv + 1] = b; }
-      __syncthreads();
-      if (lane == 0 && team_wave == 0 && !idle) {
-        double x = 0.0, y = 0.0;
-        for (int w = 0; w < team_n; ++w) { x += red[2 * (wv + w)]; y += red[2 * (wv + w) + 1]; }
-        partials[2 * (size_t)tix] = x; partials[2 * (size_t)tix + 1] = y;
-      }
-    } else {
-      block_reduce2(a, b, red);
-      if (tid == 0) { partials[2 * (size_t)tix] = a; partials[2 * (size_t)tix + 1] = b; }
-    }
-  }
+      constexpr int R = 1;
+#include "kernels_apply.hip"
+    }
+  }
+#undef SD_TILED_BODY_PASS
 #if SD_PACK_TRACE
   if constexpr (PACK) {
     if (dm.pack_trace && tid == 0 && blockIdx.y == 0) {
@@ -1057,3 +636,459 @@
   }
   return SD_OK;
 }
+
+#else
+  V own[R];
+  uint32_t sig[R];
+  typedef unsigned int u4 __attribute__((ext_vector_type(4)));
+  u4 pt[PK ? R : 1];
+  uint32_t dg[R];
+  const uint32_t off0 = (uint32_t)i0 * ES;
+  {
+    const __amdgpu_buffer_rsrc_t rs = make_rsrc(psi + base, (uint32_t)len * ES);
+#pragma unroll
+    for (int r = 0; r < R; ++r) buf_load(own[r], rs, off0 + (uint32_t)(r * 64) * ES);
+    if (PK && !need_sig && !dm.diag_cache) {
+      const __amdgpu_buffer_rsrc_t rg = make_rsrc(dm.suf_dg + rec.suf_off, (uint32_t)len);
+#pragma unroll
+      for (int r = 0; r < R; ++r) dg[r] = (uint32_t)(unsigned char)__builtin_amdgcn_raw_buffer_load_b8(rg, (uint32_t)i0 + (uint32_t)(r * 64), 0, 0);
+    }
+    if (need_sig) {
+      const __amdgpu_buffer_rsrc_t rsig = make_rsrc(dm.suf_states + rec.suf_off, (uint32_t)len * 2u);
+#pragma unroll
+      for (int r = 0; r < R; ++r) sig[r] = buf_load_u16(rsig, (uint32_t)i0 * 2u + (uint32_t)(r * 64) * 2u);
+    } else {
+#pragma unroll
+      for (int r = 0; r < R; ++r) sig[r] = 0;
+    }
+  }
+
+  uint64_t fmask = 0;
+  int64_t my_base = -1;
+  const uint32_t bitp = p >= 1 ? ((P >> (p - 1)) & 1u) : 0u;
+  if (nn > 0 && p >= 1 && !(PACK && idle)) {
+    const int b = lane + 1;
+    if (b <= p) my_base = dm.far_base[(size_t)tix * (size_t)p + (size_t)lane];
+    fmask = __ballot(my_base >= 0);
+  }
+  const int st_lo = bitp ? nU : 0, st_n = bitp ? len - nU : nU;
+  auto get_bond = [&](int ln) {
+    FarBond fb;
+    fb.base = rl64(my_base, ln); fb.J = hop_amp<PACK>(dm.hop_J, ln);
+    const bool st = ln == p - 1;
+    fb.lo = st ? st_lo : 0; fb.n = st ? st_n : len;
+    return fb;
+  };
+  constexpr bool SKIP_DEAD = NC == 1 || BLOCK == 64;
+  uint32_t live = 0;
+  if (SKIP_DEAD) {
+#pragma unroll
+    for (int r = 0; r < R; ++r)
+      if ((tid & ~63) / 64 * WR + r * 64 < len) live |= 1u << r;
+    live = (uint32_t)__builtin_amdgcn_readfirstlane((int)live);
+  }
+  auto issue = [&](const FarBond &fb, V(&v)[R]) {
+    const V *__restrict__ pb = (halo && fb.base >= dm.n_local) ? halo + (fb.base - dm.n_local) : psi + fb.base;
+    const __amdgpu_buffer_rsrc_t rs = make_rsrc(pb, (uint32_t)fb.n * ES);
+    const uint32_t rel = off0 - (uint32_t)fb.lo * ES;
+#pragma unroll
+    for (int r = 0; r < R; ++r)
+      if (!SKIP_DEAD || ((live >> r) & 1u)) buf_load(v[r], rs, rel + (uint32_t)(r * 64) * ES);
+  };
+
+  V va[R], vb[R];
+  if (SKIP_DEAD) {
+#pragma unroll
+    for (int r = 0; r < R; ++r) { va[r] = V{}; vb[r] = V{}; }
+  }
+  FarBond fa{}, fbb{};
+  uint64_t mk = fmask;
+  bool have_a = false;
+  auto next_lane = [&](uint64_t &m_) { const int ln = __builtin_ctzll(m_); m_ &= m_ - 1; return ln; };
+  constexpr int D = PACK ? SD_PACK_RING : 2;
+  u4 rq[D][R];
+  FarBond fr[D];
+  int ring_full = 0, ring_rem = 0;
+  auto ring_next = [&]() {
+    FarBond fb;
+    const bool e = mk == 0;
+    const int ln = e ? 0 : __builtin_ctzll(mk);
+    mk &= mk - 1;
+    fb.base = e ? 0 : rl64(my_base, ln);
+    fb.J = 0.0;
+    if (!e) fb.J = hop_amp<PACK>(dm.hop_J, ln);
+    const bool st = ln == p - 1;
+    fb.lo = st ? st_lo : 0; fb.n = e ? 0 : st ? st_n : len;
+    return fb;
+  };
+  auto ring_issue = [&](const FarBond &fb, u4(&v)[R]) {
+    const __amdgpu_buffer_rsrc_t rs = make_rsrc(psi + fb.base, (uint32_t)fb.n * ES);
+    const uint32_t rel = off0 - (uint32_t)fb.lo * ES;
+#pragma unroll
+    for (int r = 0; r < R; ++r) v[r] = __builtin_amdgcn_raw_buffer_load_b128(rs, rel + (uint32_t)(r * 64) * ES, 0, 0);
+  };
+  auto request_table = [&]() {
+    if (PK && (PACK || nn > 0)) {
+      const __amdgpu_buffer_rsrc_t rp = make_rsrc(dm.suf_part + 4 * (size_t)rec.suf_off, nn > 0 ? (uint32_t)len * 16u : 0u);
+#pragma unroll
+      for (int r = 0; r < R; ++r) pt[PK ? r : 0] = __builtin_amdgcn_raw_buffer_load_b128(rp, (uint32_t)i0 * 16u + (uint32_t)(r * 64) * 16u, 0, 0);
+    }
+  };
+  double dd[R];
+  auto load_dd = [&]() {
+    const __amdgpu_buffer_rsrc_t rd = make_rsrc(dm.diag_cache + base, (uint32_t)len * (uint32_t)sizeof(double));
+#pragma unroll
+    for (int r = 0; r < R; ++r) buf_load(dd[r], rd, (uint32_t)i0 * (uint32_t)sizeof(double) + (uint32_t)(r * 64) * (uint32_t)sizeof(double));
+  };
+  if constexpr (PACK) {
+    if (dm.diag_cache) load_dd();
+    request_table();
+    const int nf = __popcll(fmask);
+    const int ring_more = nf > D ? nf - D : 0;
+    ring_full = ring_more / D;
+    ring_rem = ring_more - ring_full * D;
+    FarBond fe[D];
+#pragma unroll
+    for (int j = 0; j < D; ++j) fe[j] = ring_next();
+#pragma unroll
+    for (int k = 0; k < D; ++k) {
+      fr[k] = fe[k];
+#pragma unroll
+      for (int t = 1; t < D; ++t)
+        if (ring_rem == t) fr[k] = fe[(k + t) % D];
+      ring_issue(fr[k], rq[k]);
+    }
+  } else {
+    if (mk) { fa = get_bond(next_lane(mk)); issue(fa, va); have_a = true; }
+  }
+
+  V acc[R];
+  if (dm.diag_cache) {
+    if constexpr (!PACK) load_dd();
+#pragma unroll
+    for (int r = 0; r < R; ++r) acc[r] = vscale(dd[r], own[r]);
+  } else if (!need_sig) {
+    const int antiP = p >= 2 ? __popc((P ^ (P >> 1)) & ((1u << (p - 1)) - 1u)) : 0;
+#pragma unroll
+    for (int r = 0; r < R; ++r) {
+      int anti = antiP + (int)(dg[r] & 15u) + (p >= 1 ? (int)(bitp ^ (dg[r] >> 4)) : 0);
+      if (dm.n_zz_nn == 0) anti = 0;
+      acc[r] = vscale(dm.diag_q * (double)(dm.n_zz - 2 * anti), own[r]);
+    }
+  } else if (dm.diag_mode == 0) {
+    const DiagHead dh = diag_head(dm, P, p);
+#pragma unroll
+    for (int r = 0; r < R; ++r) {
+      const uint64_t s = (uint64_t)P | ((uint64_t)sig[r] << p);
+      acc[r] = vscale(diag_tail(dm, dh, s, p), own[r]);
+    }
+  } else {
+#pragma unroll
+    for (int r = 0; r < R; ++r) {
+      const uint64_t s = (uint64_t)P | ((uint64_t)sig[r] << p);
+      acc[r] = vscale(diag_of(dm, s), own[r]);
+    }
+  }
+#pragma unroll
+  for (int r = 0; r < R; ++r)
+    if (i0 + r * 64 < len) tile[1 + i0 + r * 64] = own[r];
+  if (PACK ? (lane == 0 && team_wave == 0) : (tid == 0)) tile[0] = V{};
+  if (!PK)
+    for (int k = tid; k < 16 * SD_BIN_STRIDE; k += BLOCK) {
+      int n = k / SD_BIN_STRIDE, kk = k - n * SD_BIN_STRIDE;
+      lbin[k] = (int)binom_g(dm, n, kk);
+    }
+
+  __syncthreads();
+  if constexpr (PACK) {
+    auto ring_acc = [&](int k) {
+#pragma unroll
+      for (int r = 0; r < R; ++r) {
+        const u4 q = rq[k][r];
+        V v;
+        if constexpr (NC == 2) { v.x = __hiloint2double((int)q.y, (int)q.x); v.y = __hiloint2double((int)q.w, (int)q.z); }
+        acc[r] = accum<FMA>(acc[r], fr[k].J, v);
+      }
+    };
+    auto ring_step = [&](int k) {
+      const FarBond nb = get_bond(next_lane(mk));
+      ring_acc(k);
+      __builtin_amdgcn_sched_barrier(0);
+      fr[k] = nb;
+      ring_issue(fr[k], rq[k]);
+      __builtin_amdgcn_sched_barrier(0);
+    };
+#pragma unroll
+    for (int k = 1; k < D; ++k)
+      if (ring_rem >= D - k) ring_step(k);
+#pragma nounroll
+    for (int it = 0; it < ring_full; ++it) {
+#pragma unroll
+      for (int k = 0; k < D; ++k) ring_step(k);
+    }
+#pragma unroll
+    for (int k = 0; k < D; ++k) ring_acc(k);
+  } else {
+    while (have_a) {
+      bool have_b = false;
+      if (mk) { fbb = get_bond(next_lane(mk)); issue(fbb, vb); have_b = true; }
+#pragma unroll
+      for (int r = 0; r < R; ++r) acc[r] = accum<FMA>(acc[r], fa.J, va[r]);
+      have_a = false;
+      if (!have_b) break;
+      if (mk) { fa = get_bond(next_lane(mk)); issue(fa, va); have_a = true; }
+#pragma unroll
+      for (int r = 0; r < R; ++r) acc[r] = accum<FMA>(acc[r], fbb.J, vb[r]);
+    }
+  }
+  if constexpr (!PACK) request_table();
+  const bool wrap = !GEN && !PACK && PK && !(NC == 1 && R == 8) && nn > 0 && dm.wrap_hop == nn;
+  bool wrap_on = false;
+  if (wrap) {
+    const uint32_t Q = P ^ (1u << dm.wrap_pb);
+    const int t2q = dm.nup - __popc(Q);
+    if (t2q >= 0 && t2q <= LS) {
+      wrap_on = true;
+      const int64_t qb = dm.addr[Q];
+      const int lenq = (int)dm.binom[LS * (SD_MAX_L + 1) + t2q];
+      const V *__restrict__ pbq = (halo && qb >= dm.n_local) ? halo + (qb - dm.n_local) : psi + qb;
+      const __amdgpu_buffer_rsrc_t rq = make_rsrc(pbq, (uint32_t)lenq * ES);
+      for (int c0 = 0; c0 < lenq; c0 += BLOCK * R) {
+#pragma unroll
+        for (int r = 0; r < R; ++r) buf_load(va[r], rq, off0 + (uint32_t)(c0 + r * 64) * ES);
+#pragma unroll
+        for (int r = 0; r < R; ++r)
+          if (c0 + i0 + r * 64 < lenq) tile2[1 + c0 + i0 + r * 64] = va[r];
+      }
+      if (tid == 0) tile2[0] = V{};
+    }
+  }
+
+  struct GBond { int64_t base; uint32_t smask; int pb; int kind; };
+  auto gbond = [&](int h) {
+    GBond g{0, 0u, 0, -1};
+    const int bi = dm.hop_i[h] - 1, bj = dm.hop_j[h] - 1;
+    const bool ip = bi < p, jp = bj < p;
+    if (ip && jp) {
+      if (((P >> bi) ^ (P >> bj)) & 1u) { g.kind = 0; g.base = dm.addr[P ^ (1u << bi) ^ (1u << bj)]; }
+    } else if (!ip && !jp) {
+      g.kind = 1; g.smask = (1u << (bi - p)) | (1u << (bj - p));
+    } else {
+      g.pb = ip ? bi : bj;
+      g.smask = 1u << ((ip ? bj : bi) - p);
+      const uint32_t Q = P ^ (1u << g.pb);
+      const int t2q = dm.nup - __popc(Q);
+      if (t2q >= 0 && t2q <= LS) { g.kind = 2; g.base = dm.addr[Q]; }
+    }
+    return g;
+  };
+  auto gflip = [&](const GBond &g, int r) -> bool {
+    if (g.kind == 0) return true;
+    if (g.kind == 1) return __popc(sig[r] & g.smask) == 1;
+    if (g.kind == 2) return ((P >> g.pb) & 1u) != ((sig[r] & g.smask) ? 1u : 0u);
+    return false;
+  };
+  auto gvalue = [&](const GBond &g, int r) -> V {
+    if (g.kind == 1) return tile[1 + dm.suf_rank[sig[r] ^ g.smask]];
+    const int64_t idx = g.base + (g.kind == 0 ? (int64_t)(i0 + r * 64) : (int64_t)dm.suf_rank[sig[r] ^ g.smask]);
+    return (halo && idx >= dm.n_local) ? halo[idx - dm.n_local] : psi[idx];
+  };
+  const bool have_g = !GEN && nn < dm.n_hop;
+  double gJ = 0.0;
+  GBond g0{0, 0u, 0, -1};
+  auto request_g0 = [&]() {
+    g0 = gbond(nn);
+    gJ = dm.hop_J[nn];
+#pragma unroll
+    for (int r = 0; r < R; ++r) va[r] = (i0 + r * 64 < len && gflip(g0, r)) ? gvalue(g0, r) : V{};
+  };
+  if (have_g && !PK) request_g0();
+  if (nn > 0) {
+    if constexpr (PK) {
+      const unsigned char *tb = reinterpret_cast<const unsigned char *>(tile);
+      constexpr uint32_t SH = NC == 2 ? 4 : 3;
+#pragma unroll
+      for (int a = 1; a <= 11; ++a) if (a <= LS - 1) {
+        const double J = hop_amp<PACK>(dm.hop_J, p + a - 1);
+        const int w = (a - 1) / 3, sh = 10 * ((a - 1) % 3);
+        V v[R];
+#pragma unroll
+        for (int r = 0; r < R; ++r) {
+          const u4 q = pt[PK ? r : 0];
+          const uint32_t word = w == 0 ? q.x : w == 1 ? q.y : w == 2 ? q.z : q.w;
+          const uint32_t ad = ((word >> sh) & 0x3FFu) << SH;
+          v[r] = *reinterpret_cast<const V *>(tb + ad);
+        }
+#pragma unroll
+        for (int r = 0; r < R; ++r) acc[r] = accum<FMA>(acc[r], J, v[r]);
+      }
+    } else {
+      uint32_t dw[R];
+#pragma unroll
+      for (int r = 0; r < R; ++r) dw[r] = sig[r] ^ (sig[r] >> 1);
+      for (int a = 1; a <= LS - 1; ++a) {
+        const double J = dm.hop_J[p + a - 1];
+        const int *brow = lbin + (LS - a - 1) * SD_BIN_STRIDE;
+        int d[R];
+#pragma unroll
+        for (int r = 0; r < R; ++r) d[r] = brow[__popc(sig[r] >> (a + 1))];
+        V v[R];
+#pragma unroll
+        for (int r = 0; r < R; ++r) {
+          const bool up = (sig[r] >> (a - 1)) & 1u;
+          const bool fl = (dw[r] >> (a - 1)) & 1u;
+          const int ip = (i0 + r * 64) + (up ? d[r] : -d[r]);
+          v[r] = tile[fl ? ip + 1 : 0];
+        }
+#pragma unroll
+        for (int r = 0; r < R; ++r) acc[r] = accum<FMA>(acc[r], J, v[r]);
+      }
+    }
+  }
+  if constexpr (GEN) {
+    constexpr uint32_t SH = NC == 2 ? 4 : 3;
+    const unsigned char *tb = reinterpret_cast<const unsigned char *>(tile);
+    const unsigned char *tb2 = reinterpret_cast<const unsigned char *>(tile2);
+    uint32_t ptw[R];
+    int cur_word = -1;
+    auto gissue = [&](int64_t gbase, V(&v)[R]) {
+      const V *__restrict__ pbp = (halo && gbase >= dm.n_local) ? halo + (gbase - dm.n_local) : psi + gbase;
+      const __amdgpu_buffer_rsrc_t rs = make_rsrc(pbp, (uint32_t)len * ES);
+#pragma unroll
+      for (int r = 0; r < R; ++r) buf_load(v[r], rs, off0 + (uint32_t)(r * 64) * ES);
+    };
+    for (int hb = 0; hb < dm.n_gen; hb += 64) {
+      const int nb = dm.n_gen - hb < 64 ? dm.n_gen - hb : 64;
+      int64_t base_k = -1;
+      sd_gbond gl{-1, 0u, 0, 0, 0.0};
+      if (lane < nb) {
+        gl = dm.gen[hb + lane];
+        if (gl.kind == 0 && __popc(P & gl.pmask) == 1) base_k = dm.addr[P ^ gl.pmask];
+      }
+      uint64_t todo = __ballot(base_k >= 0);
+      int in_a = -1;
+      if (todo) { in_a = next_lane(todo); gissue(rl64(base_k, in_a), va); }
+#pragma nounroll
+      for (int k = 0; k < nb; ++k) {
+        sd_gbond gb;
+        gb.kind = rl(gl.kind, k); gb.pmask = (uint32_t)rl((int)gl.pmask, k); gb.slot = rl(gl.slot, k); gb.pb = rl(gl.pb, k);
+        gb.J = rld(gl.J, k);
+        if (gb.kind == 0) {
+          if (k == in_a) {
+#pragma unroll
+            for (int r = 0; r < R; ++r) acc[r] = accum<false>(acc[r], gb.J, va[r]);
+            in_a = -1;
+            if (todo) { in_a = next_lane(todo); gissue(rl64(base_k, in_a), va); }
+          }
+        } else if (gb.kind == 1) {
+          const int wi = gb.slot / 3, sh = 10 * (gb.slot - 3 * wi);
+          if (wi != cur_word) {
+            cur_word = wi;
+            const int chunk = wi >> 2;
+            const __amdgpu_buffer_rsrc_t rp2 = make_rsrc(dm.gen_ss_part + 4 * ((size_t)chunk * (size_t)dm.n_suf_rows + (size_t)rec.suf_off), (uint32_t)len * 16u);
+            const uint32_t wo = (uint32_t)(wi & 3) * 4u;
+#pragma unroll
+            for (int r = 0; r < R; ++r) ptw[r] = (uint32_t)__builtin_amdgcn_raw_buffer_load_b32(rp2, (uint32_t)i0 * 16u + (uint32_t)(r * 64) * 16u + wo, 0, 0);
+          }
+          V v[R];
+#pragma unroll
+          for (int r = 0; r < R; ++r) v[r] = *reinterpret_cast<const V *>(tb + ((((ptw[r] >> sh) & 0x3FFu)) << SH));
+#pragma unroll
+          for (int r = 0; r < R; ++r) acc[r] = accum<false>(acc[r], gb.J, v[r]);
+        } else if (gb.kind == 2) {
+          const uint32_t Q = P ^ gb.pmask;
+          const int t2q = dm.nup - __popc(Q);
+          const bool ok = t2q >= 0 && t2q <= LS;
+          __syncthreads();
+          if (ok) {
+            const int64_t qb = dm.addr[Q];
+            const int lenq = (int)dm.binom[LS * (SD_MAX_L + 1) + t2q];
+            const V *__restrict__ pbq = (halo && qb >= dm.n_local) ? halo + (qb - dm.n_local) : psi + qb;
+            const __amdgpu_buffer_rsrc_t rq = make_rsrc(pbq, (uint32_t)lenq * ES);
+            for (int c0 = 0; c0 < lenq; c0 += BLOCK * R) {
+              V tmp[R];
+#pragma unroll
+              for (int r = 0; r < R; ++r) buf_load(tmp[r], rq, off0 + (uint32_t)(c0 + r * 64) * ES);
+#pragma unroll
+              for (int r = 0; r < R; ++r)
+                if (c0 + i0 + r * 64 < lenq) tile2[1 + c0 + i0 + r * 64] = tmp[r];
+            }
+            if (tid == 0) tile2[0] = V{};
+          }
+          __syncthreads();
+          if (ok) {
+            const __amdgpu_buffer_rsrc_t rm = make_rsrc(dm.mix_part + ((size_t)gb.slot * (size_t)dm.n_suf_rows + (size_t)rec.suf_off), (uint32_t)len * 2u);
+            const uint32_t bpb = (P >> gb.pb) & 1u;
+            uint32_t w16[R];
+#pragma unroll
+            for (int r = 0; r < R; ++r) w16[r] = buf_load_u16(rm, (uint32_t)i0 * 2u + (uint32_t)(r * 64) * 2u);
+#pragma unroll
+            for (int r = 0; r < R; ++r) {
+              const bool has = (w16[r] >> 15) != bpb;
+              const uint32_t ad = has ? ((w16[r] & 0x3FFu) << SH) : 0u;
+              acc[r] = accum<false>(acc[r], gb.J, *reinterpret_cast<const V *>(tb2 + ad));
+            }
+          }
+        }
+      }
+    }
+  }
+  if (wrap) {
+    __syncthreads();
+    if (wrap_on) {
+      const double Jw = dm.hop_J[nn];
+      const uint32_t bpb = (P >> dm.wrap_pb) & 1u;
+      const unsigned char *tb2 = reinterpret_cast<const unsigned char *>(tile2);
+      constexpr uint32_t SH = NC == 2 ? 4 : 3;
+#pragma unroll
+      for (int r = 0; r < R; ++r) {
+        const uint32_t w3 = pt[PK ? r : 0].w;
+        const bool has = ((w3 >> 30) & 1u) != bpb;
+        const uint32_t ad = has ? (((w3 >> 20) & 0x3FFu) << SH) : 0u;
+        acc[r] = accum<false>(acc[r], Jw, *reinterpret_cast<const V *>(tb2 + ad));
+      }
+    }
+  }
+  if (have_g) {
+    if (!wrap) {
+      if (PK) request_g0();
+#pragma unroll
+      for (int r = 0; r < R; ++r)
+        if (gflip(g0, r)) acc[r] = accum<false>(acc[r], gJ, va[r]);
+    }
+    for (int h = nn + 1; h < dm.n_hop; ++h) {
+      const GBond g = gbond(h);
+      if (g.kind < 0) continue;
+      const double J = dm.hop_J[h];
+#pragma unroll
+      for (int r = 0; r < R; ++r)
+        if (i0 + r * 64 < len && gflip(g, r)) acc[r] = accum<false>(acc[r], J, gvalue(g, r));
+    }
+  }
+
+  EpiSums sums{0.0, 0.0};
+#pragma unroll
+  for (int r = 0; r < R; ++r) {
+    const int i = i0 + r * 64;
+    if (i < len) epilogue<NC>(epi, ea, base + i, acc[r], tile[1 + i], out_, sums);
+  }
+  if (epi_has_sums(epi)) {
+    double a = sums.s0, b = sums.s1;
+    if constexpr (PACK) {
+      for (int off = 32; off > 0; off >>= 1) {
+        a += __shfl_down(a, off, 64);
+        b += __shfl_down(b, off, 64);
+      }
+      if (lane == 0) { red[2 * wv] = a; red[2 * wv + 1] = b; }
+      __syncthreads();
+      if (lane == 0 && team_wave == 0 && !idle) {
+        double x = 0.0, y = 0.0;
+        for (int w = 0; w < team_n; ++w) { x += red[2 * (wv + w)]; y += red[2 * (wv + w) + 1]; }
+        partials[2 * (size_t)tix] = x; partials[2 * (size_t)tix + 1] = y;
+      }
+    } else {
+      block_reduce2(a, b, red);
+      if (tid == 0) { partials[2 * (size_t)tix] = a; partials[2 * (size_t)tix + 1] = b; }
+    }
+  }
+#endif
```

Result: no change. 106.2 (median of 6 runs) (+0.6%).
